# 0xPolygonZero/proof-protocol-decoder

Measured on NVIDIA B200. Metric: mpt_nodes_keccak_hashed_per_sec, higher is better.
Workload: dtype u64

## Files before the change

proof_protocol_decoder_b200/csrc/gpu_txn.cu:

```cuda
#include "host_pipeline.h"
#include "txn_tables.h"

namespace ppd {

bool gpu_txn_enabled() {
#ifdef PPD_HOSTPROF
  return false;
#else
  return gpu_parse_enabled() && gpu_dump_enabled() && getenv("PPD_HOST_TXN") == nullptr;
#endif
}

struct LoopBatcher {
  static const int MAX_STREAMS = 16, BMAX = (int)LOOP_BATCH_MAX;
  struct Req {
    txn::LoopTask task;
    uint32_t n_txns = 0;
    cudaEvent_t ready = nullptr, start = nullptr, done = nullptr, done_blocking = nullptr;
    bool launched = false;
    uint32_t launches = 0;
    cudaError_t err = cudaSuccess;
  };
  struct LoopStream {
    cudaStream_t st = nullptr;
    cudaEvent_t idle = nullptr;
    txn::LoopTask* tasks = nullptr;
  };
  int device = 0, n_streams = 0;
  LoopStream ls[MAX_STREAMS];
  std::mutex mu;
  std::condition_variable cv_work, cv_launched;
  std::deque<Req*> q;
  bool stop = false;
  std::thread th;

  void serve() {
#ifndef PPD_HOSTPROF
    cudaSetDevice(device);
    int next = 0;
    for (;;) {
      Req* batch[BMAX];
      int n = 0;
      {
        std::unique_lock<std::mutex> g(mu);
        cv_work.wait(g, [&] { return stop || !q.empty(); });
        if (stop && q.empty()) return;
      }
      int pick = -1;
      for (int k = 0; k < n_streams && pick < 0; k++) {
        const int s = (next + k) % n_streams;
        if (cudaEventQuery(ls[s].idle) == cudaSuccess) pick = s;
      }
      if (pick < 0) {
        pick = next;
        cudaEventSynchronize(ls[pick].idle);
      }
      next = (pick + 1) % n_streams;
      {
        std::lock_guard<std::mutex> g(mu);
        while (n < BMAX && !q.empty()) batch[n++] = q.front(), q.pop_front();
      }
      LoopStream& S = ls[pick];
      uint32_t max_txns = 0;
      bool any_shared = false;
      cudaError_t err = cudaSuccess;
      for (int k = 0; k < n; k++) {
        S.tasks[k] = batch[k]->task;
        max_txns = std::max(max_txns, batch[k]->n_txns);
        any_shared |= batch[k]->task.use_shared != 0;
        if (err == cudaSuccess) err = cudaStreamWaitEvent(S.st, batch[k]->ready, 0);
      }
      for (int k = 0; k < n && err == cudaSuccess; k++) err = cudaEventRecord(batch[k]->start, S.st);
      uint32_t launches = 0;
      if (err == cudaSuccess) {
        launches = launch_txn_loops(S.tasks, (uint32_t)n, max_txns, any_shared, S.st);
        err = cudaGetLastError();
      }
      for (int k = 0; k < n && err == cudaSuccess; k++) {
        err = cudaEventRecord(batch[k]->done, S.st);
        if (err == cudaSuccess) err = cudaEventRecord(batch[k]->done_blocking, S.st);
      }
      if (err == cudaSuccess) err = cudaEventRecord(S.idle, S.st);
      {
        std::lock_guard<std::mutex> g(mu);
        for (int k = 0; k < n; k++) batch[k]->launched = true, batch[k]->launches = launches, batch[k]->err = err;
      }
      cv_launched.notify_all();
    }
#endif
  }
};

LoopBatcher* loop_batcher_create(int device, int n_streams) {
#ifdef PPD_HOSTPROF
  return nullptr;
#else
  LoopBatcher* b = new LoopBatcher();
  b->device = device;
  b->n_streams = std::min(n_streams, (int)LoopBatcher::MAX_STREAMS);
  for (int k = 0; k < b->n_streams; k++) {
    LoopBatcher::LoopStream& S = b->ls[k];
    S.tasks = (txn::LoopTask*)pinned_alloc(sizeof(txn::LoopTask) * LoopBatcher::BMAX);
    if (!S.tasks || cudaStreamCreateWithFlags(&S.st, cudaStreamNonBlocking) != cudaSuccess ||
        cudaEventCreateWithFlags(&S.idle, cudaEventBlockingSync | cudaEventDisableTiming) != cudaSuccess || cudaEventRecord(S.idle, S.st) != cudaSuccess) {
      b->n_streams = k + 1;
      loop_batcher_destroy(b);
      return nullptr;
    }
  }
  b->th = std::thread([b] { b->serve(); });
  return b;
#endif
}
void loop_batcher_destroy(LoopBatcher* b) {
#ifndef PPD_HOSTPROF
  if (!b) return;
  if (b->th.joinable()) {
    {
      std::lock_guard<std::mutex> g(b->mu);
      b->stop = true;
    }
    b->cv_work.notify_all();
    b->th.join();
  }
  for (int k = 0; k < b->n_streams; k++) {
    if (b->ls[k].st) cudaStreamSynchronize(b->ls[k].st), cudaStreamDestroy(b->ls[k].st);
    if (b->ls[k].idle) cudaEventDestroy(b->ls[k].idle);
    if (b->ls[k].tasks) pinned_free(b->ls[k].tasks);
  }
  delete b;
#endif
}
uint32_t loop_batcher_run(LoopBatcher* b, const txn::View& v, uint32_t initial_state, uint32_t max_keys, cudaEvent_t ready, cudaEvent_t start,
                          cudaEvent_t done, cudaEvent_t done_blocking) {
#ifdef PPD_HOSTPROF
  return 0;
#else
  LoopBatcher::Req r;
  r.task.v = v, r.task.initial_state = initial_state, r.task.use_shared = txn_loop_uses_shared(max_keys);
  r.n_txns = v.n_txns, r.ready = ready, r.start = start, r.done = done, r.done_blocking = done_blocking;
  {
    std::lock_guard<std::mutex> g(b->mu);
    b->q.push_back(&r);
  }
  b->cv_work.notify_one();
  {
    std::unique_lock<std::mutex> g(b->mu);
    b->cv_launched.wait(g, [&] { return r.launched; });
  }
  CUDA_OK(r.err);
  return r.launches;
#endif
}

#ifndef PPD_HOSTPROF
namespace {

struct Carve2 {
  uint8_t* base;
  size_t off = 0;
  template <class T>
  T* take(size_t count) {
    off = (off + 255) & ~(size_t)255;
    T* r = reinterpret_cast<T*>(base + off);
    off += count * sizeof(T);
    return r;
  }
};

struct HookState {
  Lane* L;
  Job* J;
  TxnTables* T;
  const uint8_t* d_flat;
  size_t n_txns;
  TxnBases B{};
  txn::View v{};
  txn::JoinView j{};
  txn::AcctInit ai{};
  uint32_t table_slots = 0, n_pre_nodes = 0, cap_tail = 0;
  uint64_t* se = nullptr;
  uint32_t *bins_pre = nullptr, *bins_tail = nullptr;
  uint16_t* okeys = nullptr;
  txn::Withdrawal* d_withdrawals = nullptr;
  txn::AcctExport* d_export = nullptr;
  uint32_t* h_bins = nullptr;
  uint8_t* h_code_digests = nullptr;
};

void after_emit(void* arg, const ParseEmit& E) {
  HookState& H = *(HookState*)arg;
  Lane* L = H.L;
  Job& J = *H.J;
  TxnTables& T = *H.T;
  cudaStream_t st = L->st;
  const size_t n_nodes = J.dev.nodes, n_acct = J.dev.accounts, n_traces = T.traces.size();
  H.n_pre_nodes = (uint32_t)n_nodes;
  H.cap_tail = (uint32_t)T.est_nodes;
  TxnBases& B = H.B;
  B.dig_base = (uint32_t)((J.dev.keys + 31) & ~(size_t)31);
  B.txn_key_base = B.dig_base + 32u * T.n_msgs;
  B.key_cursor = B.txn_key_base + 12u * (uint32_t)H.n_txns;
  B.val_base = (uint32_t)((J.dev.vals + 3) & ~(size_t)3);
  B.rec_base = (uint32_t)n_acct;
  uint32_t table = 64;
  while (table < 2 * n_traces) table <<= 1;
  uint32_t jtable = 64;
  while (jtable < 2 * n_acct) jtable <<= 1;
  H.table_slots = table;
  txn::View& v = H.v;
  txn::JoinView& j = H.j;
  const size_t n_sorted = std::max<size_t>(n_nodes, T.est_nodes);
  const size_t pc_slow_n = (size_t)T.max_ops * txn::PATH_CAP;
  size_t pc_map_n = 64;
  while (pc_map_n < 2 * pc_slow_n) pc_map_n <<= 1;
  auto layout = [&](Carve2& c) {
    v.traces = c.take<txn::TxnTrace>(n_traces + 1);
    H.se = c.take<uint64_t>(2ull * T.n_msgs + 2);
    v.ops1 = c.take<txn::SOp>(T.n_ops1 + 1);
    v.ops2 = c.take<txn::SOp>(T.n_ops2 + 1);
    v.acct = c.take<txn::AcctState>(table);
    j.slot_owner = c.take<uint32_t>(jtable);
    j.slot_best = c.take<uint32_t>(jtable);
    j.join_storage = c.take<uint32_t>(n_acct + 1);
    j.join_root = c.take<uint32_t>(n_acct + 1);
    j.pre_flags = c.take<uint8_t>(n_acct + 1);
    v.pre_slot = c.take<uint32_t>(n_acct + 1);
    H.d_withdrawals = c.take<txn::Withdrawal>(T.withdrawals.size() + 1);
    H.d_export = c.take<txn::AcctExport>(T.needs_dummies() ? n_acct + 1 : 1);
    v.s.path_node = c.take<uint32_t>((size_t)T.max_ops * txn::PATH_CAP + 1);
    v.s.path_pc = c.take<uint32_t>((size_t)T.max_ops * txn::PATH_CAP + 1);
    v.s.path_depth = c.take<uint8_t>((size_t)T.max_ops * txn::PATH_CAP + 1);
    v.s.plen = c.take<uint8_t>(T.max_ops + 1);
    v.s.tnode = c.take<uint32_t>(T.max_ops + 1);
    v.s.tpc = c.take<uint32_t>(T.max_ops + 1);
    v.s.tdepth = c.take<uint8_t>(T.max_ops + 1);
    v.s.tkind = c.take<uint8_t>(T.max_ops + 1);
    v.s.key_hi = c.take<uint32_t>(T.max_ops + 1);
    v.s.pc_slow = c.take<txn::PathNode>(pc_slow_n + 1);
    v.s.pc_map = c.take<uint32_t>(pc_map_n);
    v.s.pc_map_key = c.take<uint32_t>(pc_map_n);
    v.cur = c.take<txn::Cursors>(1);
    H.bins_pre = c.take<uint32_t>(ORDER_MAX_BINS);
    H.bins_tail = c.take<uint32_t>(ORDER_MAX_BINS);
    H.okeys = c.take<uint16_t>(n_sorted + 16);
  };
  {
    Carve2 sz{nullptr};
    layout(sz);
    L->d_txn.reserve(sz.off + 256);
    Carve2 c{L->d_txn.as<uint8_t>()};
    layout(c);
  }
  v.nodes = E.nodes, v.level = E.level, v.key_pool = E.key_pool, v.val_pool = E.val_pool, v.hash_pool = E.hash_pool;
  v.child_pool = E.child_pool, v.accounts = E.accounts;
  v.cap_nodes = (uint32_t)(n_nodes + T.est_nodes), v.cap_children = (uint32_t)(J.dev.children + T.est_children);
  v.cap_keys = (uint32_t)std::min<size_t>(L->d_keys.cap, 0xfffffff0u);
  v.flat = H.d_flat, v.n_txns = (uint32_t)H.n_txns, v.n_traces = (uint32_t)n_traces, v.dig_base = B.dig_base;
  v.rec_base = B.rec_base, v.val_base = B.val_base;
  v.pre_flags = j.pre_flags;
  v.s.pc_fast = nullptr, v.s.pc_n_fast = 0, v.s.pc_n_slow = (uint32_t)pc_slow_n, v.s.pc_map_mask = (uint32_t)pc_map_n - 1, v.s.pc_count = &v.cur->pc_count;
  v.s.sh_ops = nullptr;
  v.s.a_nodes = &v.cur->n_nodes, v.s.a_children = &v.cur->n_children, v.s.a_keys = &v.cur->key_bytes, v.s.a_max_level = &v.cur->max_level;
  v.withdrawals = H.d_withdrawals, v.n_withdrawals = (uint32_t)T.withdrawals.size();
  lane_copy(L, H.d_withdrawals, T.withdrawals.data(), sizeof(txn::Withdrawal) * v.n_withdrawals);
  j.acct_list = E.acct_list, j.n_acct = (uint32_t)n_acct, j.table_mask = jtable - 1;
  lane_copy(L, v.traces, T.traces.data(), sizeof(txn::TxnTrace) * n_traces);
  lane_copy_flush(L);
  L->stats.h2d_bytes += (double)(sizeof(txn::TxnTrace) * n_traces);
  launch_txn_msgs(v, H.se, st);
  launch_keccak256_ranges(H.d_flat, H.se, T.n_msgs, E.key_pool + B.dig_base, st);
  L->stats.kernel_launches += 2, L->stats.key_hashes += T.n_msgs;
  for (size_t k = 0; k < T.code_write_traces.size(); k++) {
    const uint32_t m = T.traces[T.code_write_traces[k]].m_code;
    lane_copy(L, H.h_code_digests + 32 * k, E.key_pool + B.dig_base + 32ull * m, 32);
  }
  L->d_order.reserve(4ull * n_nodes + 16);
  CUDA_OK(cudaMemsetAsync(H.bins_pre, 0, 4ull * ORDER_MAX_BINS, st));
  launch_order_by_level_class(E.nodes, E.level, (uint32_t)n_nodes, ORDER_MAX_BINS, H.okeys, H.bins_pre, L->d_order.as<uint32_t>(), st);
  lane_copy(L, H.h_bins, H.bins_pre, 4ull * ORDER_MAX_BINS);
  L->stats.kernel_launches += 3, L->stats.d2h_bytes += 4.0 * ORDER_MAX_BINS;
}

void levels_from_bins(const uint32_t* bins, uint32_t n, std::vector<uint32_t>& level_start) {
  level_start.assign(1, 0);
  for (uint32_t l = 0; l < ORDER_MAX_BINS / 64; l++) {
    const uint32_t end = bins[64 * l + 63];
    level_start.push_back(end);
    if (end >= n) break;
  }
}

}
#endif

int gpu_block(ppd_ctx* c, Lane* L, Job& J, const uint8_t* flat, size_t len, uint8_t** out, size_t* out_len) {
#ifdef PPD_HOSTPROF
  return GPU_BLOCK_DECLINED;
#else
  BlockJob& b = J.blocks[0];
  if (!gpu_txn_enabled()) return GPU_BLOCK_DECLINED;
  {
    const char* e = getenv("PPD_GPU_PARSE_MIN_BYTES");
    const size_t min_bytes = e ? (size_t)atoll(e) : (size_t)512 << 10;
    if (b.compact.n < min_bytes || b.compact.n < 2) return GPU_BLOCK_DECLINED;
  }
  TxnTables& T = J.txn;
  PhaseTimer pt;
  if (!txn_tables_phase1(b, flat, len, T)) return GPU_BLOCK_DECLINED;
  pt.lap("t:tables1");
  cudaStream_t st = L->st;
  const ppd_stats stats0 = L->stats;
  const size_t wit_off = (size_t)(b.compact.p - flat);
  const size_t lead = (256 - (wit_off & 255)) & 255;
  L->d_flat.reserve(lead + len + 512);
  uint8_t* d_flat = L->d_flat.as<uint8_t>() + lead;
  L->tr_n = 0;
  trace_mark(L, "begin");
  upload_bytes(L, J, d_flat, flat, len);
  trace_mark(L, "uploaded");
  CUDA_OK(cudaMemsetAsync(d_flat + len, 0, 256, st));
  L->stats.h2d_bytes += (double)len;
  const size_t h_words = 2 * ORDER_MAX_BINS + sizeof(txn::Cursors) / 4 + 64;
  J.txn_host.resize(h_words + 8 * T.code_write_traces.size() + 8);
  HookState H;
  H.L = L, H.J = &J, H.T = &T, H.d_flat = d_flat, H.n_txns = b.txns.size();
  H.h_bins = J.txn_host.data();
  H.h_code_digests = reinterpret_cast<uint8_t*>(J.txn_host.data() + h_words);
  PreImageDeviceOnly X{};
  X.d_witness = d_flat + wit_off;
  X.extra_nodes = T.est_nodes, X.extra_children = T.est_children;
  X.extra_keys = 64 + 32ull * T.n_msgs + 12ull * b.txns.size() + 40ull * (T.n_ops1 + T.n_ops2) + 4096;
  X.extra_vals = 64 + T.val_writes + 8ull * b.txns.size();
  for (const TxnV& tx : b.txns) X.extra_vals += tx.byte_code.n + tx.new_receipt_node.n;
  X.extra_accounts = T.n_recs + 1;
  X.after_launch = after_emit, X.arg = &H;
  if (!gpu_pre_image(L, J, b, true, &c->parse_slots_sem, &X)) {
    L->stats = stats0;
    return GPU_BLOCK_DECLINED;
  }
  pt.lap("t:pre-image");
  trace_mark(L, "parsed");
  struct CD {
    HookState* H;
    TxnTables* T;
    std::vector<uint32_t> slot_of;
  } cd{&H, &T, {}};
  if (!T.code_write_traces.empty()) {
    cd.slot_of.assign(T.traces.size(), 0);
    for (size_t k = 0; k < T.code_write_traces.size(); k++) cd.slot_of[T.code_write_traces[k]] = (uint32_t)k;
  }
  auto code_digest = [](void* arg, uint32_t t) -> const uint8_t* {
    CD* x = (CD*)arg;
    return x->H->h_code_digests + 32ull * x->slot_of[t];
  };
  if (!txn_tables_phase2(b, flat, H.B, code_digest, &cd, T)) {
    L->stats = stats0;
    return GPU_BLOCK_DECLINED;
  }
  pt.lap("t:tables2");
  txn::View& v = H.v;
  const uint32_t n_ir = T.n_ir, n_seg = (uint32_t)T.seg_a.size(), n_touched = T.touched_begin[n_ir];
  const uint32_t n_pre = H.n_pre_nodes;
  const int n_dummies = (T.dummy_initial[0] >= 0) + (T.dummy_initial[1] >= 0) + (T.dummy_final >= 0);
  const size_t dummy_entries = J.dev.accounts + T.traces.size();
  const size_t seg_cap = n_seg + (size_t)n_dummies * (2 * dummy_entries + 32), lit_cap = T.lit.size() + (size_t)n_dummies * (36 * dummy_entries + 512);
  PVec<uint64_t>& big_off = J.big_off;
  PVec<uint32_t>& big_cap = J.big_cap;
  big_off.resize(n_ir + 1), big_cap.resize(n_ir + 1);
  size_t big_words = 0;
  for (uint32_t i = 0; i < n_ir; i++) {
    const uint32_t tn = T.touched_begin[i + 1] - T.touched_begin[i];
    big_off[i] = ~0ull, big_cap[i] = 0;
    if (tn <= 2 * IR_SET_MAX_UNIQ) continue;
    uint32_t cap = 1u << 14;
    while (cap < 2 * tn) cap <<= 1;
    big_off[i] = big_words, big_cap[i] = cap;
    big_words += 3ull * cap;
  }
  IrDumpPlanView P{};
  uint64_t* d_big_off;
  uint32_t* d_big_cap;
  uint32_t *d_seg_a, *d_seg_b, *d_seg_c, *d_seg_begin, *d_seg_end, *d_touched_begin, *d_touched, *d_ir_size;
  uint64_t* d_ir_base;
  uint8_t* d_lit;
  txn::TxnDesc* d_txns;
  auto plan_layout = [&](Carve2& cv) {
    d_txns = cv.take<txn::TxnDesc>(n_ir + 1);
    d_seg_a = cv.take<uint32_t>(seg_cap + 1), d_seg_b = cv.take<uint32_t>(seg_cap + 1), d_seg_c = cv.take<uint32_t>(seg_cap + 1);
    d_seg_begin = cv.take<uint32_t>(n_ir + 1), d_seg_end = cv.take<uint32_t>(n_ir + 1), d_touched_begin = cv.take<uint32_t>(n_ir + 1);
    d_lit = cv.take<uint8_t>(lit_cap + 16);
    d_ir_base = cv.take<uint64_t>(n_ir + 1);
    d_touched = cv.take<uint32_t>((size_t)n_touched + 16);
    P.seg_off = cv.take<uint32_t>(seg_cap + 1);
    d_ir_size = cv.take<uint32_t>(2ull * n_ir + 2);
    P.ir_nuniq = cv.take<uint32_t>(n_ir + 1);
    d_big_off = cv.take<uint64_t>(n_ir + 1), d_big_cap = cv.take<uint32_t>(n_ir + 1);
    P.big_scratch = cv.take<uint32_t>(big_words + 16);
    P.u_node = cv.take<uint32_t>((size_t)n_touched + 16), P.u_size = cv.take<uint32_t>((size_t)n_touched + 16), P.u_off = cv.take<uint32_t>((size_t)n_touched + 16);
  };
  {
    Carve2 sz{nullptr};
    plan_layout(sz);
    L->d_plan.reserve(sz.off + 256);
    Carve2 cv{L->d_plan.as<uint8_t>()};
    plan_layout(cv);
  }
  P.ir_size = d_ir_size, P.ir_flag = d_ir_size + n_ir;
  P.touched = d_touched, P.touched_begin = d_touched_begin, P.seg_a = d_seg_a, P.seg_b = d_seg_b, P.seg_c = d_seg_c, P.seg_begin = d_seg_begin;
  P.seg_end = d_seg_end;
  P.big_off = d_big_off, P.big_cap = d_big_cap;
  P.flat = d_flat, P.lit = d_lit, P.ir_base = d_ir_base;
  auto up = [&](void* dst, const void* src, size_t bytes) {
    if (!bytes) return;
    lane_copy(L, dst, src, bytes);
    L->stats.h2d_bytes += (double)bytes;
  };
  up(d_txns, T.txns.data(), sizeof(txn::TxnDesc) * T.txns.size());
  up(d_seg_a, T.seg_a.data(), 4ull * n_seg), up(d_seg_b, T.seg_b.data(), 4ull * n_seg), up(d_seg_c, T.seg_c.data(), 4ull * n_seg);
  up(d_touched_begin, T.touched_begin.data(), 4ull * (n_ir + 1));
  if (!n_dummies) up(d_seg_begin, T.seg_begin.data(), 4ull * (n_ir + 1)), up(d_seg_end, T.seg_end.data(), 4ull * (n_ir + 1));
  up(d_lit, T.lit.data(), T.lit.size());
  up(d_big_off, big_off.data(), 8ull * n_ir), up(d_big_cap, big_cap.data(), 4ull * n_ir);
  up(v.key_pool + H.B.txn_key_base, T.txn_keys.data(), T.txn_keys.size());
  lane_copy_flush(L);
  CUDA_OK(cudaMemsetAsync(d_touched, 0xff, 4ull * n_touched, st));
  v.txns = d_txns, v.touched = d_touched, v.seg_a = d_seg_a, v.seg_b = d_seg_b;
  std::vector<uint32_t> level_pre, level_tail;
  levels_from_bins(H.h_bins, n_pre, level_pre);
  L->d_ref.reserve(32ull * v.cap_nodes);
  L->d_ref_len.reserve(v.cap_nodes);
  L->d_counters.reserve(32);
  CUDA_OK(cudaMemsetAsync(L->d_counters.p, 0, 32, st));
  ArenaView V;
  V.nodes = v.nodes, V.key_pool = v.key_pool, V.val_pool = v.val_pool, V.hash_pool = v.hash_pool, V.child_pool = v.child_pool;
  V.accounts = v.accounts, V.ref = L->d_ref.as<uint8_t>(), V.ref_len = L->d_ref_len.as<uint8_t>();
  V.counters = L->d_counters.as<unsigned long long>();
  trace_mark(L, "plan_up");
  CUDA_OK(cudaEventRecord(L->ev0, st));
  for (size_t l = 0; l + 1 < level_pre.size(); l++) {
    launch_hash_level(V, L->d_order.as<uint32_t>(), level_pre[l], level_pre[l + 1], st);
    L->stats.kernel_launches++, L->stats.level_launches++;
  }
  CUDA_OK(cudaEventRecord(L->ev1, st));
  trace_mark(L, "pre_hashed");
  H.j.ref = V.ref;
  CUDA_OK(cudaMemsetAsync(H.j.slot_owner, 0xff, 4ull * (H.j.table_mask + 1), st));
  CUDA_OK(cudaMemsetAsync(H.j.slot_best, 0, 4ull * (H.j.table_mask + 1), st));
  CUDA_OK(cudaMemsetAsync(v.pre_slot, 0xff, 4ull * (H.j.n_acct + 1), st));
  txn::Cursors init;
  memset(&init, 0, sizeof init);
  init.n_nodes = n_pre, init.n_children = (uint32_t)J.dev.children, init.key_bytes = H.B.key_cursor;
  init.state_root = b.state_root, init.txn_root = NODE_EMPTY, init.receipt_root = NODE_EMPTY;
  launch_txn_init(v, init, H.table_slots, st);
  H.j.flag = &v.cur->flag;
  launch_join(H.j, st);
  H.ai = txn::AcctInit{H.table_slots - 1, b.state_root, H.j.join_storage, H.j.join_root};
  const uint32_t max_writes = T.max_trace_keys;
  L->stats.kernel_launches += 3 + launch_txn_prep(v, H.ai, T.n_ops1, T.n_ops2, max_writes, st);
#ifdef PPD_LOOP_PROF
  static unsigned long long* d_evlog = nullptr;
  static uint32_t* d_evcount = nullptr;
  const uint32_t ev_cap = 1u << 16;
  const char* ev_env = getenv("PPD_LOOP_EVLOG");
  if (ev_env) {
    if (!d_evlog) {
      CUDA_OK(cudaMalloc(&d_evlog, 16ull * ev_cap));
      CUDA_OK(cudaMalloc(&d_evcount, 4));
    }
    CUDA_OK(cudaMemsetAsync(d_evcount, 0, 4, st));
    v.evlog = d_evlog, v.evcount = d_evcount, v.ev_txn = (uint32_t)atoi(ev_env), v.ev_cap = ev_cap;
  }
#endif
  trace_mark(L, "prep");
  lane_copy_flush(L);
  CUDA_OK(cudaEventRecord(L->ev_ready, st));
  L->lease->release();
  L->stats.kernel_launches += loop_batcher_run(c->batcher, v, b.state_root, T.max_ops, L->ev_ready, L->ev_loop0, L->ev_loop1, L->ev_loop_done);
  {
    const auto tw = std::chrono::steady_clock::now();
    CUDA_OK(cudaEventSynchronize(L->ev_loop_done));
    L->stats.host_wait_ms += std::chrono::duration<double, std::milli>(std::chrono::steady_clock::now() - tw).count();
  }
  L->lease->acquire();
  st = L->st;
  trace_mark(L, "loop");
  L->d_order2.reserve(4ull * H.cap_tail + 16);
  CUDA_OK(cudaMemsetAsync(H.bins_tail, 0, 4ull * ORDER_MAX_BINS, st));
  launch_order_by_level_class(v.nodes, v.level, H.cap_tail, ORDER_MAX_BINS, H.okeys, H.bins_tail, L->d_order2.as<uint32_t>(), st, n_pre, &v.cur->n_nodes);
  CUDA_OK(cudaGetLastError());
  txn::Cursors* h_cur = reinterpret_cast<txn::Cursors*>(H.h_bins + 2 * ORDER_MAX_BINS);
  lane_copy(L, H.h_bins + ORDER_MAX_BINS, H.bins_tail, 4ull * ORDER_MAX_BINS);
  lane_copy(L, h_cur, v.cur, sizeof(txn::Cursors));
  L->stats.kernel_launches += 3, L->stats.d2h_bytes += 4.0 * ORDER_MAX_BINS + sizeof(txn::Cursors);
  trace_mark(L, "tail_order");
  lane_sync(L);
  pt.lap("t:loop");
#ifdef PPD_LOOP_PROF
  if (ev_env && strchr(ev_env, ':')) {
    uint32_t n_ev = 0;
    CUDA_OK(cudaMemcpy(&n_ev, d_evcount, 4, cudaMemcpyDeviceToHost));
    n_ev = std::min(n_ev, ev_cap);
    std::vector<unsigned long long> ev(2ull * n_ev);
    if (n_ev) CUDA_OK(cudaMemcpy(ev.data(), d_evlog, 16ull * n_ev, cudaMemcpyDeviceToHost));
    if (FILE* f = fopen(strchr(ev_env, ':') + 1, "w")) {
      fprintf(f, "clock,thread,event\n");
      for (uint32_t k = 0; k < n_ev; k++) fprintf(f, "%llu,%llu,%llu\n", ev[2 * k], ev[2 * k + 1] >> 16, ev[2 * k + 1] & 0xffff);
      fclose(f);
    }
  }
#endif
  {
    float ms = 0;
    CUDA_OK(cudaEventElapsedTime(&ms, L->ev0, L->ev1));
    L->stats.gpu_ms += ms;
    CUDA_OK(cudaEventElapsedTime(&ms, L->ev_loop0, L->ev_loop1));
    L->stats.txn_gpu_ms += ms;
  }
  if (getenv("PPD_TIMING")) {
    const unsigned long long* pc = h_cur->phase_clocks;
    fprintf(stderr, "[ppd]   loop phases (Mclk): setup %.2f | walks %.2f | announce %.2f | storage tries up %.2f | records %.2f | state trie up %.2f | root nodes %.2f\n",
            pc[0] / 1e6, pc[1] / 1e6, pc[2] / 1e6, pc[3] / 1e6, pc[4] / 1e6, pc[5] / 1e6, pc[6] / 1e6);
  }
  if (h_cur->flag || h_cur->max_level >= ORDER_MAX_BINS / 64) {
    if (getenv("PPD_TIMING")) fprintf(stderr, "[ppd] device txn loop flag %u at txn %u (max level %u): host path\n", h_cur->flag, h_cur->flag_txn, h_cur->max_level);
    L->stats = stats0;
    L->has_last_parse = false;
    return GPU_BLOCK_DECLINED;
  }
  if (n_dummies) {
    const size_t n_acct = J.dev.accounts, n_tr = T.traces.size();
    const size_t w_export = (sizeof(txn::AcctExport) * (n_acct + 1) + 3) / 4, w_table = (sizeof(txn::AcctState) * H.table_slots + 3) / 4, w_dig = 8 * (n_tr + 1);
    J.txn_export.resize(w_export + w_table + w_dig + 16);
    txn::AcctExport* h_export = reinterpret_cast<txn::AcctExport*>(J.txn_export.data());
    txn::AcctState* h_table = reinterpret_cast<txn::AcctState*>(J.txn_export.data() + w_export);
    uint8_t* h_dig = reinterpret_cast<uint8_t*>(J.txn_export.data() + w_export + w_table);
    launch_acct_export(v, H.j, H.d_export, st);
    CUDA_OK(cudaGetLastError());
    lane_copy(L, h_export, H.d_export, sizeof(txn::AcctExport) * n_acct);
    lane_copy(L, h_table, v.acct, sizeof(txn::AcctState) * H.table_slots);
    lane_copy(L, h_dig, v.key_pool + H.B.dig_base, 32ull * n_tr);
    L->stats.kernel_launches += 1, L->stats.d2h_bytes += (double)(sizeof(txn::AcctExport) * n_acct + sizeof(txn::AcctState) * H.table_slots + 32ull * n_tr);
    lane_sync(L);
    const size_t seg0 = T.seg_a.size(), lit0 = T.lit.size();
    txn_tables_dummies(b, flat, *h_cur, h_export, (uint32_t)n_acct, h_table, H.table_slots, h_dig, T);
    if (T.seg_a.size() > seg_cap || T.lit.size() > lit_cap) fail(PPD_ERR_BAD_ARGUMENT, "dummy entries exceed their plan space");
    up(d_seg_a + seg0, T.seg_a.data() + seg0, 4ull * (T.seg_a.size() - seg0)), up(d_seg_b + seg0, T.seg_b.data() + seg0, 4ull * (T.seg_b.size() - seg0));
    up(d_seg_c + seg0, T.seg_c.data() + seg0, 4ull * (T.seg_c.size() - seg0));
    up(d_lit + lit0, T.lit.data() + lit0, T.lit.size() - lit0);
    up(d_seg_begin, T.seg_begin.data(), 4ull * (n_ir + 1)), up(d_seg_end, T.seg_end.data(), 4ull * (n_ir + 1));
    lane_copy_flush(L);
    pt.lap("t:dummies");
  }
  const uint32_t n_total = h_cur->n_nodes, n_tail = n_total - n_pre;
  levels_from_bins(H.h_bins + ORDER_MAX_BINS, n_tail, level_tail);
  trace_mark(L, "host_resumed");
  CUDA_OK(cudaEventRecord(L->ev0, st));
  for (size_t l = 0; l + 1 < level_tail.size(); l++) {
    launch_hash_level(V, L->d_order2.as<uint32_t>(), level_tail[l], level_tail[l + 1], st);
    L->stats.kernel_launches++, L->stats.level_launches++;
  }
  CUDA_OK(cudaEventRecord(L->ev1, st));
  trace_mark(L, "tail_hashed");
  CUDA_OK(cudaEventRecord(L->ev_loop0, st));
  launch_ir_size(V, P, n_ir, st);
  CUDA_OK(cudaEventRecord(L->ev_loop1, st));
  CUDA_OK(cudaGetLastError());
  J.plan.resize(2ull * n_ir + 8);
  uint32_t* h_sizes = J.plan.data();
  unsigned long long* h_counters = reinterpret_cast<unsigned long long*>(H.h_bins);
  lane_copy(L, h_sizes, d_ir_size, 8ull * n_ir);
  lane_copy(L, h_counters, L->d_counters.p, 24);
  L->stats.kernel_launches += 1, L->stats.d2h_bytes += 8.0 * n_ir + 24;
  trace_mark(L, "ir_sized");
  lane_sync(L);
  pt.lap("t:sweep+size");
  {
    float ms = 0;
    CUDA_OK(cudaEventElapsedTime(&ms, L->ev0, L->ev1));
    L->stats.gpu_ms += ms;
    CUDA_OK(cudaEventElapsedTime(&ms, L->ev_loop0, L->ev_loop1));
    L->stats.dump_gpu_ms += ms;
  }
  L->stats.nodes_hashed += h_counters[0], L->stats.node_permutations += h_counters[1], L->stats.node_bytes += h_counters[2];
  L->stats.arena_nodes += n_total;
  L->stats.levels += level_pre.size() + level_tail.size() - 2;
  for (size_t m = 0; m < T.traces.size(); m++) {
    const txn::TxnTrace& tr = T.traces[m];
    L->stats.key_permutations += 1 + tr.n_reads + tr.n_writes + ((tr.flags & txn::TRF_MIN_KEYS) ? tr.n_writes : 0);
    if ((tr.flags & PPD_TR_CODE_WRITE) && !(tr.flags & PPD_TR_CODE_READ)) L->stats.key_permutations += tr.code_len / 136 + 1;
  }
  L->stats.marks_on_gpu += T.n_items;
  L->stats.txn_loops_on_gpu += 1;
  L->has_last = true, L->last_view = V;
  L->last_level_start = level_pre, L->last_level_start2 = level_tail, L->last_n_msgs = T.n_msgs;
  L->last_msg_data = d_flat, L->last_msg_se = H.se, L->last_digest_out = v.key_pool + H.B.dig_base;
  L->last_txn = H.v, L->last_join = H.j, L->last_ai = H.ai, L->last_init = init, L->last_table_slots = H.table_slots;
  L->last_n_ops1 = T.n_ops1, L->last_n_ops2 = T.n_ops2, L->last_max_writes = max_writes, L->last_n_touched = n_touched, L->last_max_keys = T.max_ops;
  L->last_plan = P, L->last_n_ir = n_ir, L->has_last_txn = true;
  L->last_cap_tail = H.cap_tail, L->last_bins_tail = H.bins_tail, L->last_okeys = H.okeys;
  uint64_t total = 8;
  PVec<uint64_t>& ir_base = J.ir_base;
  ir_base.resize(n_ir);
  for (uint32_t i = 0; i < n_ir; i++) {
    if (h_sizes[n_ir + i]) {
      if (getenv("PPD_TIMING")) fprintf(stderr, "[ppd] IR %u cannot be laid out on the device: host path\n", i);
      L->stats = stats0;
      L->has_last = L->has_last_parse = L->has_last_txn = false;
      return GPU_BLOCK_DECLINED;
    }
    ir_base[i] = total;
    total += h_sizes[i];
  }
  Out o;
  uint8_t* pinned = total >= ((size_t)1 << 20) ? out_pool().take(total) : nullptr;
  if (!pinned) o.need(total);
  uint8_t* dst = pinned ? pinned : o.p;
  L->d_out.reserve(total + 64);
  L->last_out_bytes = total;
  up(d_ir_base, ir_base.data(), 8ull * n_ir);
  launch_store_u32x2(L->d_out.as<uint32_t>(), PPD_IR_DUMP_MAGIC, n_ir, st);
  L->stats.h2d_bytes += 8;
  lane_copy_flush(L);
  trace_mark(L, "host_resumed2");
  CUDA_OK(cudaEventRecord(L->ev0, st));
  launch_ir_emit(V, P, n_ir, L->d_out.as<uint8_t>(), st);
  CUDA_OK(cudaEventRecord(L->ev1, st));
  trace_mark(L, "ir_emitted");
  CUDA_OK(cudaGetLastError());
  L->stats.kernel_launches += 1;
  if (pinned) {
    const auto tw = std::chrono::steady_clock::now();
    cudaError_t e = cudaMemcpyAsync(dst, L->d_out.p, total, cudaMemcpyDeviceToHost, st);
    trace_mark(L, "downloaded");
    if (e == cudaSuccess) e = cudaEventRecord(L->ev_sync, st);
    if (e == cudaSuccess) e = cudaEventSynchronize(L->ev_sync);
    L->stats.host_wait_ms += std::chrono::duration<double, std::milli>(std::chrono::steady_clock::now() - tw).count();
    if (e != cudaSuccess) {
      out_pool().give_back(pinned);
      throw Fail{PPD_ERR_CUDA, std::string("IR dump copy: ") + cudaGetErrorString(e)};
    }
  } else {
    J.out_stage.resize(total);
    CUDA_OK(cudaMemcpyAsync(J.out_stage.data(), L->d_out.p, total, cudaMemcpyDeviceToHost, st));
    lane_sync(L);
    memcpy(o.p, J.out_stage.data(), total);
    o.n = total;
  }
  L->stats.d2h_bytes += (double)total;
  {
    float ms = 0;
    CUDA_OK(cudaEventElapsedTime(&ms, L->ev0, L->ev1));
    L->stats.dump_gpu_ms += ms;
  }
  pt.lap("t:emit+copy");
  trace_mark(L, "end");
  trace_flush(L);
  if (pinned) {
    *out = pinned, *out_len = total;
  } else {
    *out = o.give(out_len);
  }
  return GPU_BLOCK_DONE;
#endif
}

}
```

proof_protocol_decoder_b200/csrc/host_pipeline.h:

```cpp
#pragma once
#include <cuda_runtime.h>
#include <sys/mman.h>

#include <algorithm>
#include <atomic>
#include <chrono>
#include <condition_variable>
#include <cstdio>
#include <cstdlib>
#include <cstring>
#include <deque>
#include <map>
#include <memory>
#include <mutex>
#include <string>
#include <thread>
#include <unordered_set>
#include <unordered_map>
#include <vector>

#include "../../include/ppd_b200.h"
#include "arena.h"
#include "devbuf.h"
#include "flat_maps.h"
#include "host_arena.h"
#include "ppd_kernels.h"
#include "txn_tables.h"

namespace ppd {

static const uint8_t EMPTY_CODE_HASH[32] = {0xc5, 0xd2, 0x46, 0x01, 0x86, 0xf7, 0x23, 0x3c, 0x92, 0x7e, 0x7d, 0xb2, 0xdc, 0xc7, 0x03, 0xc0,
                                            0xe5, 0x00, 0xb6, 0x53, 0xca, 0x82, 0x27, 0x3b, 0x7b, 0xfa, 0xd8, 0x04, 0x5d, 0x85, 0xa4, 0x70};
static const uint8_t EMPTY_TRIE_HASH[32] = {0x56, 0xe8, 0x1f, 0x17, 0x1b, 0xcc, 0x55, 0xa6, 0xff, 0x83, 0x45, 0xe6, 0x92, 0xc0, 0xf8, 0x6e,
                                            0x5b, 0x48, 0xe0, 0x1b, 0x99, 0x6c, 0xad, 0xc0, 0x01, 0x62, 0x2f, 0xb5, 0xe3, 0x63, 0xb4, 0x21};

struct Job;
void job_delete(Job*);
void* pinned_alloc(size_t n);
void pinned_free(void* p);

struct Lane {
  cudaStream_t st = nullptr;
  cudaEvent_t ev0 = nullptr, ev1 = nullptr;
  cudaEvent_t ev_sync = nullptr;
  ppd_stats stats{};
  DevBuf d_nodes, d_order, d_keys, d_vals, d_hashes, d_children, d_accounts, d_ref, d_ref_len, d_counters;
  DevBuf d_msg, d_msg_off, d_digest;
  DevBuf d_plan, d_out;
  DevBuf d_wit, d_pa, d_pb, d_pc;
  DevBuf d_level, d_okeys, d_obins;
  DevBuf d_flat, d_txn, d_order2;
  cudaEvent_t ev_loop0 = nullptr, ev_loop1 = nullptr;
  uint32_t* h_parse = nullptr;
  bool has_last_parse = false;
  ParseBounds last_bounds{};
  ParseEmit last_emit{};
  uint32_t* last_ins_pos = nullptr;
  uint32_t last_n_code = 0;
  size_t last_val_bytes = 0;
  Job* job = nullptr;
  bool has_last = false;
  ArenaView last_view{};
  std::vector<uint32_t> last_level_start, last_level_start2;
  uint32_t last_n_msgs = 0;
  const uint8_t* last_msg_data = nullptr;
  const uint64_t* last_msg_se = nullptr;
  uint8_t* last_digest_out = nullptr;
  bool has_last_txn = false;
  txn::View last_txn{};
  txn::JoinView last_join{};
  txn::AcctInit last_ai{};
  txn::Cursors last_init{};
  uint32_t last_table_slots = 0, last_n_ops1 = 0, last_n_ops2 = 0, last_max_writes = 0, last_n_touched = 0, last_n_ir = 0, last_cap_tail = 0, last_max_keys = 0;
  uint32_t* last_bins_tail = nullptr;
  uint16_t* last_okeys = nullptr;
  IrDumpPlanView last_plan{};
  size_t last_out_bytes = 0;
  std::vector<cudaEvent_t> tr_ev;
  std::vector<const char*> tr_label;
  std::vector<double> tr_host_ms;
  size_t tr_n = 0;
  int id = 0;
  CopyBatch copies;
  cudaStream_t own_st = nullptr;
  struct StreamLease* lease = nullptr;
  txn::LoopTask* h_task = nullptr;
  cudaEvent_t ev_ready = nullptr, ev_loop_done = nullptr;
};

struct Slots {
  std::mutex mu;
  std::condition_variable cv;
  int free_slots;
  explicit Slots(int n) : free_slots(n) {}
  void acquire() {
    std::unique_lock<std::mutex> g(mu);
    cv.wait(g, [&] { return free_slots > 0; });
    free_slots--;
  }
  void release() {
    {
      std::lock_guard<std::mutex> g(mu);
      free_slots++;
    }
    cv.notify_one();
  }
};
struct SlotGuard {
  Slots* s;
  explicit SlotGuard(Slots* s_, double* wait_ms = nullptr) : s(s_) {
    if (!s) return;
    const auto t0 = std::chrono::steady_clock::now();
    s->acquire();
    if (wait_ms) *wait_ms += std::chrono::duration<double, std::milli>(std::chrono::steady_clock::now() - t0).count();
  }
  void done() {
    if (s) s->release();
    s = nullptr;
  }
  ~SlotGuard() { done(); }
};
constexpr int PARSE_SLOTS = 8;

}

namespace ppd {
struct StreamPool {
  std::mutex mu;
  std::condition_variable cv;
  std::vector<cudaStream_t> all, free_;
  cudaStream_t acquire(double* wait_ms) {
    const auto t0 = std::chrono::steady_clock::now();
    std::unique_lock<std::mutex> g(mu);
    cv.wait(g, [&] { return !free_.empty(); });
    cudaStream_t s = free_.back();
    free_.pop_back();
    if (wait_ms) *wait_ms += std::chrono::duration<double, std::milli>(std::chrono::steady_clock::now() - t0).count();
    return s;
  }
  void release(cudaStream_t s) {
    {
      std::lock_guard<std::mutex> g(mu);
      free_.push_back(s);
    }
    cv.notify_one();
  }
};
struct StreamLease {
  StreamPool* pool;
  Lane* L;
  bool held = false;
  StreamLease(StreamPool* p, Lane* l) : pool(p), L(l) {
    L->lease = this;
    acquire();
  }
  void acquire() {
    if (!pool || held) return;
    L->st = pool->acquire(&L->stats.host_wait_ms);
    held = true;
  }
  void release() {
    if (!pool || !held) return;
    lane_copy_flush_fwd(L);
    pool->release(L->st);
    L->st = L->own_st;
    held = false;
  }
  ~StreamLease() {
    release();
    L->lease = nullptr;
  }
  static void lane_copy_flush_fwd(Lane* l);
};
struct LoopBatcher;
LoopBatcher* loop_batcher_create(int device, int n_streams);
void loop_batcher_destroy(LoopBatcher* b);
uint32_t loop_batcher_run(LoopBatcher* b, const txn::View& v, uint32_t initial_state, uint32_t max_keys, cudaEvent_t ready, cudaEvent_t start,
                          cudaEvent_t done, cudaEvent_t done_blocking);
}

struct ppd_ctx {
  int device = 0;
  ppd::StreamPool* pool = nullptr;
  ppd::LoopBatcher* batcher = nullptr;
  ppd::Slots parse_slots_sem{ppd::PARSE_SLOTS};
  cudaStream_t st = nullptr;
  cudaEvent_t ev0 = nullptr, ev1 = nullptr;
  std::string err;
  std::mutex err_mu;
  ppd_stats stats{};
  std::vector<ppd::Lane*> lanes;
  size_t last_lanes_used = 0;
  ppd::DevBuf d_keys, d_vals, d_ref, d_ref_len, d_counters;
  ppd::DevBuf d_msg, d_msg_off, d_digest;
  ppd::DevBuf d_build[12];
};

namespace ppd {

void stats_reset(ppd_ctx* c);
void lane_sync(Lane* l);
void lane_copy(Lane* l, void* dst, const void* src, size_t bytes);
void lane_copy_flush(Lane* l);
bool trace_on();
void trace_mark(Lane* l, const char* label);
void trace_flush(Lane* l);

struct KeyHasher {
  PVec<uint8_t> data;
  std::vector<uint64_t> off{0};
  PVec<H256> digest;
  std::vector<uint64_t> lens;
  PVec<uint64_t> se;
  KeyHasher() {
    data.alloc_fn = pinned_alloc, data.free_fn = pinned_free;
    digest.alloc_fn = pinned_alloc, digest.free_fn = pinned_free;
    se.alloc_fn = pinned_alloc, se.free_fn = pinned_free;
  }
  void reset() {
    data.clear(), digest.clear(), lens.clear(), se.clear();
    off.assign(1, 0);
  }
  uint32_t add(const uint8_t* p, size_t n) {
    size_t at = data.size(), padded = (n + 3) & ~(size_t)3;
    data.resize(at + padded);
    memcpy(data.data() + at, p, n);
    memset(data.data() + at + n, 0, padded - n);
    uint32_t idx = (uint32_t)lens.size();
    lens.push_back(n);
    off.push_back(data.size());
    return idx;
  }
  void run(Lane* c);
};

struct Span {
  const uint8_t* p = nullptr;
  uint32_t n = 0;
};
struct WNode {
  uint32_t pos;
  uint8_t op, flags;
  uint16_t unused = 0;
  int32_t first_child;
  int32_t next_sibling;
  uint32_t aux;
};

struct WCursor {
  const uint8_t* p;
  size_t n, pos = 0;
  uint8_t read_byte() {
    if (pos >= n) fail(PPD_ERR_UNEXPECTED_END_OF_STREAM, "read_byte at end of stream");
    return p[pos++];
  }
  bool cbor_head(uint8_t& major, uint64_t& arg) {
    if (pos >= n) return false;
    uint8_t b = p[pos++];
    major = b >> 5;
    uint8_t ai = b & 31;
    if (ai < 24) {
      arg = ai;
      return true;
    }
    if (ai > 27) return false;
    size_t w = (size_t)1 << (ai - 24);
    if (n - pos < w) return false;
    arg = 0;
    for (size_t i = 0; i < w; i++) arg = (arg << 8) | p[pos++];
    return true;
  }
  Span cbor_bytes(int err) {
    uint8_t major;
    uint64_t len;
    if (!cbor_head(major, len) || major != 2 || len > n - pos) fail(err, "bad CBOR byte string");
    Span s{p + pos, (uint32_t)len};
    pos += len;
    return s;
  }
  uint64_t cbor_uint(uint64_t max) {
    uint8_t major;
    uint64_t v;
    if (!cbor_head(major, v) || major != 0 || v > max) fail(PPD_ERR_INVALID_BYTES_FOR_TYPE, "bad CBOR unsigned integer");
    return v;
  }
};

inline uint32_t compact_key_nibbles(Span k, uint8_t* out) {
  if (k.n == 0) return 0;
  uint32_t c = 0;
  if (k.n == 1) {
    out[c++] = k.p[0] & 15;
    return c;
  }
  bool odd = k.p[0] & 1;
  uint32_t m = k.n - 1;
  if (2 * m > 64 + 1) fail(PPD_ERR_KEY_ERROR, "compact key longer than 64 nibbles");
  for (uint32_t i = 0; i + 1 < m; i++) {
    out[c++] = k.p[1 + i] >> 4;
    out[c++] = k.p[1 + i] & 15;
  }
  out[c++] = k.p[m] >> 4;
  if (!odd) out[c++] = k.p[m] & 15;
  return c;
}

inline void check_key_length(Span k) {
  if (k.n >= 2 && 2 * (k.n - 1) > 64 + 1) fail(PPD_ERR_KEY_ERROR, "compact key longer than 64 nibbles");
}

struct Witness {
  const uint8_t* bytes = nullptr;
  size_t len = 0;
  uint8_t version = 0;
  std::vector<WNode> ins;
  int32_t root = -1;

  Span key(const WNode& x) const {
    WCursor c{bytes, len, x.pos};
    return c.cbor_bytes(PPD_ERR_INVALID_BYTE_VECTOR);
  }
  Span leaf_value(const WNode& x) const {
    WCursor c{bytes, len, x.pos};
    c.cbor_bytes(PPD_ERR_INVALID_BYTE_VECTOR);
    return c.cbor_bytes(PPD_ERR_INVALID_BYTE_VECTOR);
  }
  Span code(const WNode& x) const { return key(x); }
  const uint8_t* hash(const WNode& x) const { return bytes + x.pos; }
  void account(const WNode& x, Span& key_out, uint64_t& nonce, Span& balance) const {
    WCursor c{bytes, len, x.pos};
    key_out = c.cbor_bytes(PPD_ERR_INVALID_BYTE_VECTOR);
    c.pos++;
    nonce = (x.flags & 4) ? c.cbor_uint(~0ull) : 0;
    balance = (x.flags & 8) ? c.cbor_bytes(PPD_ERR_INVALID_BYTE_VECTOR) : Span{};
  }
};
void parse_witness(const uint8_t* w, size_t n, Witness& out);

struct TrieItem {
  uint32_t koff, klen;
  uint8_t kind;
  uint32_t a1, a2;
};

struct TraceV {
  const uint8_t* addr;
  uint8_t flags;
  const uint8_t *balance = nullptr, *nonce = nullptr;
  uint32_t n_reads = 0, n_writes = 0;
  const uint8_t *reads = nullptr, *writes = nullptr;
  const uint8_t* code_read = nullptr;
  Span code_write;
  uint32_t m_addr = 0, m_reads = 0, m_writes_full = 0, m_writes_min = 0, m_code = 0;
};
struct TxnV {
  std::vector<TraceV> traces;
  Span byte_code, new_txn_node, new_receipt_node;
  uint64_t gas_used = 0;
};
struct FlatReader {
  const uint8_t* p;
  size_t n, pos = 0;
  void need(size_t k) {
    if (n - pos < k) fail(PPD_ERR_BAD_FLAT_INPUT, "flat block truncated");
  }
  uint8_t u8() {
    need(1);
    return p[pos++];
  }
  uint32_t u32() {
    need(4);
    uint32_t v;
    memcpy(&v, p + pos, 4);
    pos += 4;
    return v;
  }
  uint64_t u64() {
    need(8);
    uint64_t v;
    memcpy(&v, p + pos, 8);
    pos += 8;
    return v;
  }
  const uint8_t* raw(size_t k) {
    need(k);
    const uint8_t* r = p + pos;
    pos += k;
    return r;
  }
  Span bytes() {
    uint32_t k = u32();
    return Span{raw(k), k};
  }
};

struct IrPlan {
  uint64_t txn_before = 0, gas_before = 0, gas_after = 0;
  bool has_signed_txn = false;
  Span signed_txn;
  bool has_withdrawals = false;
  uint32_t state_sub = NODE_EMPTY, txn_sub = NODE_EMPTY, receipt_sub = NODE_EMPTY;
  std::vector<std::pair<H256, uint32_t>> storage_subs;
  std::vector<uint32_t> touched;
  uint32_t root_state = 0, root_txn = 0, root_receipt = 0;
  std::map<H256, Span> code;
};

struct BlockJob {
  Span compact;
  uint32_t pre_image_kind = 0;
  Span direct;
  std::vector<uint8_t> compact_owned;
  std::vector<H256> direct_keep;
  std::vector<TxnV> txns;
  std::unordered_map<H256, Span, H256Hasher> resolved_code;
  std::vector<std::pair<const uint8_t*, const uint8_t*>> withdrawals;
  std::vector<uint32_t> m_withdrawal_addr;
  const uint8_t* checkpoint = nullptr;
  Span b_meta, b_hashes;
  Witness wit;
  std::vector<uint32_t> m_inline_code;
  std::map<H256, Span> pre_code;
  uint32_t state_root = NODE_EMPTY;
  H256Map storage;
  struct PreAccount {
    H256 haddr;
    uint32_t rec;
    bool storage_nonempty;
    bool witnesses_storage = false;
    uint32_t own_root = NODE_EMPTY;
  };
  bool storage_partial = false;
  bool pre_image_built = false;
  std::vector<PreAccount> pre_accounts;
  H256Map pre_with_storage;
  FlatMapU32 root_of;
  std::unordered_map<int32_t, uint32_t> storage_root_of_instr;
  bool have_empty_form = false;
  bool pre_image_on_gpu = false;
  uint32_t empty_form = NODE_EMPTY;
  std::vector<IrPlan> irs;
  int status = PPD_OK;
  std::string err;
};

void read_flat_block(const uint8_t* p, size_t n, BlockJob& b);
void direct_to_compact(BlockJob& b);
void direct_filter_storage(BlockJob& b);
uint32_t u256_sig(const uint8_t* be);
void rlp_str(std::vector<uint8_t>& out, const uint8_t* p, size_t n);
void rlp_u256(std::vector<uint8_t>& out, const uint8_t* be);
struct RlpItem {
  bool is_list;
  const uint8_t* payload;
  size_t payload_len, total_len;
};
bool rlp_item(const uint8_t* p, size_t n, RlpItem& it);
bool is_legacy_receipt(const uint8_t* p, size_t n);

struct Job {
  HostArena A;
  KeyHasher kh;
  std::vector<BlockJob> blocks;
  PVec<uint8_t> ref, ref_len;
  PVec<uint32_t> order;
  PVec<uint32_t> plan;
  PVec<uint8_t> out_stage;
  bool refs_on_host = false;
  struct Resident {
    size_t nodes = 0, keys = 0, vals = 0, hashes = 0, children = 0, accounts = 0;
  } dev;
  bool pools_on_host = true;
  PVec<uint32_t> acct_list, code_list;
  PVec<uint8_t> wit_stage;
  std::vector<HostArena::MarkItem> mark_items;
  std::vector<HostArena::BatchItem> batch_items;
  std::vector<uint32_t> haddr_keys, haddr_leaves;
  PVec<H256> code_digest;
  TxnTables txn;
  PVec<uint32_t> txn_host;
  PVec<uint32_t> txn_export;
  PVec<uint64_t> ir_base, big_off;
  PVec<uint32_t> big_cap;
  std::vector<uint32_t> stamp;
  uint32_t serial = 0;
  Job() {
    plan.alloc_fn = pinned_alloc, plan.free_fn = pinned_free;
    out_stage.alloc_fn = pinned_alloc, out_stage.free_fn = pinned_free;
    A.set_allocator(pinned_alloc, pinned_free);
    ref.alloc_fn = ref_len.alloc_fn = pinned_alloc, ref.free_fn = ref_len.free_fn = pinned_free;
    order.alloc_fn = pinned_alloc, order.free_fn = pinned_free;
    A.level.alloc_fn = pinned_alloc, A.level.free_fn = pinned_free;
    acct_list.alloc_fn = code_list.alloc_fn = pinned_alloc, acct_list.free_fn = code_list.free_fn = pinned_free;
    code_digest.alloc_fn = pinned_alloc, code_digest.free_fn = pinned_free;
    wit_stage.alloc_fn = pinned_alloc, wit_stage.free_fn = pinned_free;
    txn.set_allocator(pinned_alloc, pinned_free);
    txn_host.alloc_fn = pinned_alloc, txn_host.free_fn = pinned_free;
    txn_export.alloc_fn = pinned_alloc, txn_export.free_fn = pinned_free;
    ir_base.alloc_fn = pinned_alloc, ir_base.free_fn = pinned_free;
    big_off.alloc_fn = pinned_alloc, big_off.free_fn = pinned_free, big_cap.alloc_fn = pinned_alloc, big_cap.free_fn = pinned_free;
  }
  void reset(size_t n_blocks) {
    dev = Resident{};
    pools_on_host = true;
    A.clear();
    kh.reset();
    blocks.clear();
    blocks.resize(n_blocks);
    ref.clear(), ref_len.clear(), order.clear();
    serial = 0;
  }
};

Job& job_of(Lane* l, size_t n_blocks);
Lane* lane_of(ppd_ctx* c, size_t w);
void lane_delete(Lane* l);
void collect_witness_messages(Job& J, BlockJob& b);
void collect_messages(Job& J, BlockJob& b);
uint32_t root_node_for(Job& J, BlockJob& b, uint32_t trie_root);
void build_pre_image(Job& J, BlockJob& b);
void join_storage_by_root(Lane* L, Job& J, BlockJob& b);
bool gpu_parse_enabled();
struct PreImageDeviceOnly {
  const uint8_t* d_witness;
  size_t extra_nodes, extra_children, extra_keys, extra_vals, extra_accounts;
  void (*after_launch)(void* arg, const ParseEmit& E);
  void* arg;
};
bool gpu_pre_image(Lane* L, Job& J, BlockJob& b, bool check_version = true, Slots* slots = nullptr, const PreImageDeviceOnly* dev_only = nullptr);
void upload_bytes(Lane* L, Job& J, uint8_t* dst, const uint8_t* src, size_t n);
void verify_gpu_pre_image(Lane* L, Job& J, BlockJob& b);
void shape_block(Job& J, BlockJob& b);
void sweep(Lane* c, Job& J, bool refs_to_host = true);
void fetch_refs(Lane* c, Job& J);
void fetch_pools(Lane* c, Job& J);

struct PhaseTimer {
  bool on = getenv("PPD_TIMING") != nullptr;
  std::chrono::steady_clock::time_point t = std::chrono::steady_clock::now();
  void lap(const char* what) {
    if (!on) return;
    auto now = std::chrono::steady_clock::now();
    fprintf(stderr, "[ppd] %-10s %8.3f ms\n", what, std::chrono::duration<double, std::milli>(now - t).count());
    t = now;
  }
};
struct SectionTimer {
  bool on = getenv("PPD_TIMING") != nullptr;
  double acc[8] = {0, 0, 0, 0, 0, 0, 0, 0};
  std::chrono::steady_clock::time_point t;
  void start() {
    if (on) t = std::chrono::steady_clock::now();
  }
  void stop(int k) {
    if (!on) return;
    auto now = std::chrono::steady_clock::now();
    acc[k] += std::chrono::duration<double, std::milli>(now - t).count();
    t = now;
  }
  void report(const char* const* names, int n) {
    if (!on) return;
    for (int k = 0; k < n; k++) fprintf(stderr, "[ppd]   %-12s %8.3f ms\n", names[k], acc[k]);
  }
};

struct Out {
  uint8_t* p = nullptr;
  size_t n = 0, cap = 0;
  Out() {}
  Out(const Out&) = delete;
  Out& operator=(const Out&) = delete;
  Out(Out&& o) noexcept : p(o.p), n(o.n), cap(o.cap) { o.p = nullptr, o.n = o.cap = 0; }
  ~Out() { free(p); }
  void need(size_t k) {
    if (n + k <= cap) return;
    size_t nc = cap ? cap * 2 : 4096;
    while (nc < n + k) nc *= 2;
    uint8_t* q;
    if (nc >= (8u << 20)) {
      nc = (nc + (2u << 20) - 1) & ~(size_t)((2u << 20) - 1);
      q = (uint8_t*)aligned_alloc(2u << 20, nc);
      if (q) {
        madvise(q, nc, MADV_HUGEPAGE);
        if (n) memcpy(q, p, n);
        free(p);
      }
    } else {
      q = (uint8_t*)realloc(p, nc);
    }
    if (!q) fail(PPD_ERR_BAD_ARGUMENT, "out of host memory");
    p = q, cap = nc;
  }
  void u8(uint8_t v) {
    need(1);
    p[n++] = v;
  }
  void u32(uint32_t v) {
    need(4);
    memcpy(p + n, &v, 4);
    n += 4;
  }
  void u64(uint64_t v) {
    need(8);
    memcpy(p + n, &v, 8);
    n += 8;
  }
  void raw(const uint8_t* q, size_t k) {
    need(k);
    if (k) memcpy(p + n, q, k);
    n += k;
  }
  void span(Span s) {
    u32(s.n);
    raw(s.p, s.n);
  }
  void u256(uint64_t v) {
    need(32);
    memset(p + n, 0, 24);
    for (int i = 0; i < 8; i++) p[n + 31 - i] = (uint8_t)(v >> (8 * i));
    n += 32;
  }
  uint8_t* give(size_t* len) {
    uint8_t* r = p ? p : (uint8_t*)malloc(1);
    *len = n;
    p = nullptr, n = cap = 0;
    return r;
  }
};

struct Stamp {
  std::vector<uint32_t> v;
  uint32_t serial = 0;
};

void dump_ir(const Job& J, const BlockJob& b, IrPlan& p, Stamp& st, Out& o);
void dump_blocks(Job& J, uint8_t** outs, size_t* out_lens, unsigned max_workers);
unsigned host_threads();

template <class F>
void parallel_for(size_t n, unsigned workers, F f) {
  if (workers > n) workers = (unsigned)n;
  if (workers <= 1) {
    for (size_t i = 0; i < n; i++) f(i, 0u);
    return;
  }
  std::atomic<size_t> next{0};
  std::atomic<bool> failed{false};
  Fail first{PPD_OK, ""};
  std::mutex mu;
  auto body = [&](unsigned w) {
    for (;;) {
      size_t i = next.fetch_add(1);
      if (i >= n || failed.load()) return;
      try {
        f(i, w);
      } catch (const Fail& e) {
        std::lock_guard<std::mutex> g(mu);
        if (!failed.exchange(true)) first = e;
      } catch (const std::exception& e) {
        std::lock_guard<std::mutex> g(mu);
        if (!failed.exchange(true)) first = Fail{PPD_ERR_BAD_ARGUMENT, e.what()};
      }
    }
  };
  std::vector<std::thread> th;
  for (unsigned w = 1; w < workers; w++) th.emplace_back(body, w);
  body(0);
  for (auto& t : th) t.join();
  if (failed.load()) throw first;
}

struct OutPool {
  struct Entry {
    uint8_t* p;
    size_t cap;
    bool in_use;
  };
  std::mutex mu;
  std::vector<Entry> entries;
  size_t total = 0;
  size_t limit() {
    static size_t v = [] {
      const char* e = getenv("PPD_PINNED_OUT_MB");
      return (size_t)(e ? atoll(e) : 12288) << 20;
    }();
    return v;
  }
  uint8_t* take(size_t n) {
#ifdef PPD_HOSTPROF
    return nullptr;
#else
    std::lock_guard<std::mutex> g(mu);
    Entry* best = nullptr;
    for (Entry& e : entries)
      if (!e.in_use && e.cap >= n && (!best || e.cap < best->cap)) best = &e;
    if (best) {
      best->in_use = true;
      return best->p;
    }
    size_t cap = (n + (n >> 3) + (8u << 20) - 1) & ~(size_t)((8u << 20) - 1);
    if (total + cap > limit()) {
      for (size_t i = 0; i < entries.size() && total + cap > limit();)
        if (!entries[i].in_use) {
          cudaFreeHost(entries[i].p);
          total -= entries[i].cap;
          entries.erase(entries.begin() + i);
        } else {
          i++;
        }
      if (total + cap > limit()) return nullptr;
    }
    void* p = nullptr;
    if (cudaHostAlloc(&p, cap, cudaHostAllocPortable) != cudaSuccess) return nullptr;
    entries.push_back({(uint8_t*)p, cap, true});
    total += cap;
    return (uint8_t*)p;
#endif
  }
  bool give_back(void* p) {
    std::lock_guard<std::mutex> g(mu);
    for (Entry& e : entries)
      if (e.p == p) {
        e.in_use = false;
        return true;
      }
    return false;
  }
};
OutPool& out_pool();

bool gpu_txn_enabled();
enum { GPU_BLOCK_DECLINED = 0, GPU_BLOCK_DONE = 1 };
int gpu_block(ppd_ctx* c, Lane* L, Job& J, const uint8_t* flat, size_t len, uint8_t** out, size_t* out_len);
bool gpu_dump_enabled();
enum { DUMP_ON_HOST = 0, DUMP_DONE = 1 };
int gpu_dump_block(ppd_ctx* c, Lane* L, Job& J, uint8_t** out, size_t* out_len);

}
```

proof_protocol_decoder_b200/csrc/ppd_host.cu:

```cuda
#include <time.h>

#include "host_pipeline.h"
#ifdef PPD_HOSTPROF
#include "../../tools/hostprof_stub.h"
#endif

using namespace ppd;

namespace ppd {

#ifdef PPD_HOSTPROF
void* pinned_alloc(size_t n) { return malloc(n); }
void pinned_free(void* p) { free(p); }
#else
void* pinned_alloc(size_t n) {
  void* p = nullptr;
  return cudaHostAlloc(&p, n, cudaHostAllocDefault) == cudaSuccess ? p : nullptr;
}
void pinned_free(void* p) { cudaFreeHost(p); }
#endif

void stats_reset(ppd_ctx* c) { c->stats = ppd_stats{}; }

void StreamLease::lane_copy_flush_fwd(Lane* l) { lane_copy_flush(l); }
void lane_copy_flush(Lane* l) {
#ifndef PPD_HOSTPROF
  if (!l->copies.n) return;
  launch_copy_segments(l->copies, l->st);
  CUDA_OK(cudaGetLastError());
  l->stats.kernel_launches += 1;
  l->copies.n = 0;
#endif
}
void lane_copy(Lane* l, void* dst, const void* src, size_t bytes) {
  if (!bytes) return;
  if (l->copies.n == CopyBatch::MAX) lane_copy_flush(l);
  CopyBatch& b = l->copies;
  b.dst[b.n] = dst, b.src[b.n] = src, b.bytes[b.n] = bytes, b.n++;
}

void lane_sync(Lane* l) {
  lane_copy_flush(l);
  const auto t0 = std::chrono::steady_clock::now();
  CUDA_OK(cudaEventRecord(l->ev_sync, l->st));
  CUDA_OK(cudaEventSynchronize(l->ev_sync));
  l->stats.host_wait_ms += std::chrono::duration<double, std::milli>(std::chrono::steady_clock::now() - t0).count();
}

namespace {
struct TraceState {
  FILE* f = nullptr;
  cudaEvent_t base = nullptr;
  std::chrono::steady_clock::time_point host0;
  std::mutex mu;
  unsigned seq = 0;
};
TraceState& trace_state() {
  static TraceState* t = [] {
    TraceState* s = new TraceState;
#ifndef PPD_HOSTPROF
    const char* path = getenv("PPD_TRACE");
    if (path && *path && (s->f = fopen(path, "w")) != nullptr) {
      if (cudaEventCreate(&s->base) != cudaSuccess || cudaEventRecord(s->base, 0) != cudaSuccess || cudaEventSynchronize(s->base) != cudaSuccess) {
        fclose(s->f);
        s->f = nullptr;
      }
      s->host0 = std::chrono::steady_clock::now();
      if (s->f) fprintf(s->f, "lane,block,label,device_ms,host_ms\n");
    }
#endif
    return s;
  }();
  return *t;
}
}
bool trace_on() { return trace_state().f != nullptr; }
void trace_mark(Lane* l, const char* label) {
#ifndef PPD_HOSTPROF
  TraceState& t = trace_state();
  if (!t.f) return;
  if (l->tr_n == l->tr_ev.size()) {
    cudaEvent_t e;
    CUDA_OK(cudaEventCreate(&e));
    l->tr_ev.push_back(e), l->tr_label.push_back(label), l->tr_host_ms.push_back(0);
  }
  CUDA_OK(cudaEventRecord(l->tr_ev[l->tr_n], l->st));
  l->tr_label[l->tr_n] = label;
  l->tr_host_ms[l->tr_n] = std::chrono::duration<double, std::milli>(std::chrono::steady_clock::now() - t.host0).count();
  l->tr_n++;
#endif
}
void trace_flush(Lane* l) {
#ifndef PPD_HOSTPROF
  TraceState& t = trace_state();
  if (!t.f || !l->tr_n) return;
  std::lock_guard<std::mutex> g(t.mu);
  const unsigned seq = t.seq++;
  for (size_t k = 0; k < l->tr_n; k++) {
    float ms = 0;
    if (cudaEventSynchronize(l->tr_ev[k]) != cudaSuccess || cudaEventElapsedTime(&ms, t.base, l->tr_ev[k]) != cudaSuccess) ms = -1;
    fprintf(t.f, "%d,%u,%s,%.4f,%.4f\n", l->id, seq, l->tr_label[k], ms, l->tr_host_ms[k]);
  }
  fflush(t.f);
  l->tr_n = 0;
#endif
}

void KeyHasher::run(Lane* c) {
  size_t n = lens.size();
  digest.resize(n);
  if (!n) return;
#ifdef PPD_HOSTPROF
  for (size_t i = 0; i < n; i++) hostprof::keccak256(data.data() + off[i], lens[i], digest[i].b);
  return;
#endif
  se.resize(2 * n);
  for (size_t i = 0; i < n; i++) se[2 * i] = off[i], se[2 * i + 1] = off[i] + lens[i];
  c->d_msg.reserve(data.size() + 16);
  c->d_msg_off.reserve(se.size() * 8);
  c->d_digest.reserve(n * 32);
  CUDA_OK(cudaMemcpyAsync(c->d_msg.p, data.data(), data.size(), cudaMemcpyHostToDevice, c->st));
  CUDA_OK(cudaMemcpyAsync(c->d_msg_off.p, se.data(), se.size() * 8, cudaMemcpyHostToDevice, c->st));
  launch_keccak256_ranges(c->d_msg.as<uint8_t>(), c->d_msg_off.as<uint64_t>(), (uint32_t)n, c->d_digest.as<uint8_t>(), c->st);
  CUDA_OK(cudaGetLastError());
  CUDA_OK(cudaMemcpyAsync(digest.data(), c->d_digest.p, n * 32, cudaMemcpyDeviceToHost, c->st));
  lane_sync(c);
  c->stats.key_hashes += n;
  for (size_t i = 0; i < n; i++) c->stats.key_permutations += lens[i] / 136 + 1;
  c->stats.h2d_bytes += (double)(data.size() + se.size() * 8);
  c->stats.d2h_bytes += (double)(n * 32);
  c->stats.kernel_launches += 1;
}

void job_delete(Job* j) { delete j; }
Job& job_of(Lane* l, size_t n_blocks) {
  if (!l->job) l->job = new Job();
  l->job->reset(n_blocks);
  return *l->job;
}

Lane* lane_of(ppd_ctx* c, size_t w) {
  while (c->lanes.size() <= w) {
    std::unique_ptr<Lane> l(new Lane());
    l->id = (int)c->lanes.size();
#ifndef PPD_HOSTPROF
    CUDA_OK(cudaStreamCreateWithFlags(&l->st, cudaStreamNonBlocking));
    l->own_st = l->st;
    l->h_task = (txn::LoopTask*)pinned_alloc(sizeof(txn::LoopTask));
    if (!l->h_task) fail(PPD_ERR_BAD_ARGUMENT, "out of page-locked memory");
    CUDA_OK(cudaEventCreateWithFlags(&l->ev_ready, cudaEventDisableTiming));
    CUDA_OK(cudaEventCreateWithFlags(&l->ev_loop_done, cudaEventBlockingSync | cudaEventDisableTiming));
    CUDA_OK(cudaEventCreate(&l->ev0));
    CUDA_OK(cudaEventCreate(&l->ev1));
    CUDA_OK(cudaEventCreateWithFlags(&l->ev_sync, cudaEventBlockingSync | cudaEventDisableTiming));
    CUDA_OK(cudaEventCreate(&l->ev_loop0));
    CUDA_OK(cudaEventCreate(&l->ev_loop1));
#endif
    c->lanes.push_back(l.release());
  }
  return c->lanes[w];
}
void lane_delete(Lane* l) {
#ifndef PPD_HOSTPROF
  DevBuf* bufs[] = {&l->d_nodes, &l->d_order,  &l->d_keys,     &l->d_vals, &l->d_hashes,  &l->d_children, &l->d_accounts,
                    &l->d_ref,   &l->d_ref_len, &l->d_counters, &l->d_msg,  &l->d_msg_off, &l->d_digest,
                    &l->d_plan,  &l->d_out,     &l->d_wit,      &l->d_pa,   &l->d_pb,      &l->d_pc,
                    &l->d_level, &l->d_okeys,   &l->d_obins,    &l->d_flat, &l->d_txn,     &l->d_order2};
  for (DevBuf* b : bufs) b->release();
  if (l->h_parse) pinned_free(l->h_parse);
  for (cudaEvent_t e : l->tr_ev) cudaEventDestroy(e);
  if (l->h_task) pinned_free(l->h_task);
  if (l->ev_ready) cudaEventDestroy(l->ev_ready);
  if (l->ev_loop_done) cudaEventDestroy(l->ev_loop_done);
  if (l->ev0) cudaEventDestroy(l->ev0);
  if (l->ev1) cudaEventDestroy(l->ev1);
  if (l->ev_sync) cudaEventDestroy(l->ev_sync);
  if (l->ev_loop0) cudaEventDestroy(l->ev_loop0);
  if (l->ev_loop1) cudaEventDestroy(l->ev_loop1);
  if (l->st) cudaStreamDestroy(l->st);
#endif
  if (l->job) job_delete(l->job);
  delete l;
}

void sweep(Lane* c, Job& J, bool refs_to_host) {
  HostArena& A = J.A;
  uint32_t n = (uint32_t)A.nodes.size();
  J.ref.resize(32ull * n);
  J.ref_len.resize(n);
  J.refs_on_host = true;
  if (!n) return;
#ifdef PPD_HOSTPROF
  memset(J.ref.data(), 0, 32ull * n);
  memset(J.ref_len.data(), 32, n);
  return;
#endif
  uint32_t n_levels = 0;
  for (uint32_t i = 0; i < n; i++) n_levels = std::max<uint32_t>(n_levels, A.level[i] + 1u);
  std::vector<uint32_t> level_start(n_levels + 1, 0);
  for (uint32_t i = 0; i < n; i++) level_start[A.level[i] + 1u]++;
  for (uint32_t l = 0; l < n_levels; l++) level_start[l + 1] += level_start[l];
  const bool device_order = 64u * n_levels <= ORDER_MAX_BINS;
  PVec<uint32_t>& order = J.order;
  if (!device_order) {
    auto node_class = [&](uint32_t i) -> uint32_t {
      const NodeRec& r = A.nodes[i];
      uint32_t kind = r.w0 & 0xff;
      if (kind == NK_BRANCH) return 40 + ((uint32_t)__builtin_popcount(r.a1 & 0xffff) - 1 & 15);
      if (kind == NK_ROOT) return 56;
      uint32_t perms = 1;
      if (kind == NK_LEAF) {
        uint32_t nl = (r.w0 >> 16) & 0xff;
        perms = ((nl < 2 ? 1 : 2 + (nl >> 1)) + r.a2 + 6) / 136 + 1;
      }
      return kind * 8 + (perms > 8 ? 7 : perms - 1);
    };
    order.resize(n);
    std::vector<uint8_t> cls(n);
    std::vector<uint32_t> bucket((size_t)n_levels * 64 + 1, 0);
    for (uint32_t i = 0; i < n; i++) {
      cls[i] = (uint8_t)node_class(i);
      bucket[(size_t)A.level[i] * 64 + cls[i] + 1]++;
    }
    for (size_t k = 0; k + 1 < bucket.size(); k++) bucket[k + 1] += bucket[k];
    for (uint32_t i = 0; i < n; i++) order[bucket[(size_t)A.level[i] * 64 + cls[i]]++] = i;
  }
  const Job::Resident& R = J.dev;
  c->d_nodes.reserve_keep(16ull * n, 16ull * R.nodes, c->st);
  c->d_order.reserve(4ull * n);
  c->d_keys.reserve_keep(A.key_pool.size() + 16, R.keys, c->st);
  c->d_vals.reserve_keep(A.val_pool.size() + 16, R.vals, c->st);
  c->d_hashes.reserve_keep(A.hash_pool.size() + 32, R.hashes, c->st);
  c->d_children.reserve_keep(4ull * A.child_pool.size() + 16, 4ull * R.children, c->st);
  c->d_accounts.reserve_keep(sizeof(AccountRec) * A.accounts.size() + 16, sizeof(AccountRec) * R.accounts, c->st);
  c->d_ref.reserve(32ull * n);
  c->d_ref_len.reserve(n);
  c->d_counters.reserve(32);
  auto up = [&](DevBuf& d, const void* src, size_t bytes, size_t resident = 0) {
    if (bytes <= resident) return;
    CUDA_OK(cudaMemcpyAsync(d.as<uint8_t>() + resident, (const uint8_t*)src + resident, bytes - resident, cudaMemcpyHostToDevice, c->st));
    c->stats.h2d_bytes += (double)(bytes - resident);
  };
  up(c->d_nodes, A.nodes.data(), 16ull * n, 16ull * R.nodes);
  if (device_order) {
    c->d_level.reserve_keep(2ull * n + 16, 2ull * R.nodes, c->st);
    c->d_okeys.reserve(2ull * n + 16);
    c->d_obins.reserve(4ull * ORDER_MAX_BINS);
    up(c->d_level, A.level.data(), 2ull * n, 2ull * R.nodes);
    CUDA_OK(cudaMemsetAsync(c->d_obins.p, 0, 4ull * 64 * n_levels, c->st));
    launch_order_by_level_class(c->d_nodes.as<NodeRec>(), c->d_level.as<uint16_t>(), n, 64 * n_levels, c->d_okeys.as<uint16_t>(),
                                c->d_obins.as<uint32_t>(), c->d_order.as<uint32_t>(), c->st);
    c->stats.kernel_launches += 3;
  } else {
    up(c->d_order, order.data(), 4ull * n);
  }
  up(c->d_keys, A.key_pool.data(), A.key_pool.size(), R.keys);
  up(c->d_vals, A.val_pool.data(), A.val_pool.size(), R.vals);
  up(c->d_hashes, A.hash_pool.data(), A.hash_pool.size(), R.hashes);
  up(c->d_children, A.child_pool.data(), 4ull * A.child_pool.size(), 4ull * R.children);
  up(c->d_accounts, A.accounts.data(), sizeof(AccountRec) * A.accounts.size(), sizeof(AccountRec) * R.accounts);
  CUDA_OK(cudaMemsetAsync(c->d_counters.p, 0, 32, c->st));
  ArenaView V;
  V.nodes = c->d_nodes.as<NodeRec>();
  V.key_pool = c->d_keys.as<uint8_t>();
  V.val_pool = c->d_vals.as<uint8_t>();
  V.hash_pool = c->d_hashes.as<uint8_t>();
  V.child_pool = c->d_children.as<uint32_t>();
  V.accounts = c->d_accounts.as<AccountRec>();
  V.ref = c->d_ref.as<uint8_t>();
  V.ref_len = c->d_ref_len.as<uint8_t>();
  V.counters = c->d_counters.as<unsigned long long>();
  CUDA_OK(cudaEventRecord(c->ev0, c->st));
  for (uint32_t l = 0; l < n_levels; l++) {
    launch_hash_level(V, c->d_order.as<uint32_t>(), level_start[l], level_start[l + 1], c->st);
    c->stats.kernel_launches++;
    c->stats.level_launches++;
  }
  CUDA_OK(cudaGetLastError());
  CUDA_OK(cudaEventRecord(c->ev1, c->st));
  unsigned long long counters[3] = {0, 0, 0};
  c->has_last = true;
  c->last_view = V;
  c->last_level_start = level_start;
  c->last_level_start2.clear();
  c->last_msg_data = nullptr;
  c->has_last_txn = false;
  c->last_n_msgs = (uint32_t)J.kh.lens.size();
  J.refs_on_host = refs_to_host;
  if (refs_to_host) {
    CUDA_OK(cudaMemcpyAsync(J.ref.data(), c->d_ref.p, 32ull * n, cudaMemcpyDeviceToHost, c->st));
    CUDA_OK(cudaMemcpyAsync(J.ref_len.data(), c->d_ref_len.p, n, cudaMemcpyDeviceToHost, c->st));
  }
  CUDA_OK(cudaMemcpyAsync(counters, c->d_counters.p, 24, cudaMemcpyDeviceToHost, c->st));
  lane_sync(c);
  float ms = 0;
  CUDA_OK(cudaEventElapsedTime(&ms, c->ev0, c->ev1));
  c->stats.gpu_ms += ms;
  c->stats.nodes_hashed += counters[0];
  c->stats.node_permutations += counters[1];
  c->stats.node_bytes += counters[2];
  c->stats.arena_nodes += n;
  c->stats.levels += n_levels;
  if (refs_to_host) c->stats.d2h_bytes += 33.0 * n;
}

void fetch_refs(Lane* c, Job& J) {
  if (J.refs_on_host) return;
  size_t n = J.A.nodes.size();
  CUDA_OK(cudaMemcpyAsync(J.ref.data(), c->d_ref.p, 32ull * n, cudaMemcpyDeviceToHost, c->st));
  CUDA_OK(cudaMemcpyAsync(J.ref_len.data(), c->d_ref_len.p, n, cudaMemcpyDeviceToHost, c->st));
  lane_sync(c);
  c->stats.d2h_bytes += 33.0 * n;
  J.refs_on_host = true;
}

void fetch_pools(Lane* c, Job& J) {
  if (J.pools_on_host) return;
  if (J.dev.vals) CUDA_OK(cudaMemcpyAsync(J.A.val_pool.data(), c->d_vals.p, J.dev.vals, cudaMemcpyDeviceToHost, c->st));
  if (J.dev.hashes) CUDA_OK(cudaMemcpyAsync(J.A.hash_pool.data(), c->d_hashes.p, J.dev.hashes, cudaMemcpyDeviceToHost, c->st));
  lane_sync(c);
  c->stats.d2h_bytes += (double)(J.dev.vals + J.dev.hashes);
  J.pools_on_host = true;
}

}

namespace {

template <class F>
int guarded(ppd_ctx* c, F f) {
  if (!c) return PPD_ERR_BAD_ARGUMENT;
  try {
#ifndef PPD_HOSTPROF
    CUDA_OK(cudaSetDevice(c->device));
#endif
    f();
    return PPD_OK;
  } catch (const Fail& e) {
    c->err = e.msg;
    return e.code;
  } catch (const std::exception& e) {
    c->err = e.what();
    return PPD_ERR_BAD_ARGUMENT;
  }
}

}

namespace ppd {
OutPool& out_pool() {
  static OutPool* p = new OutPool();
  return *p;
}
}

namespace {

void decode_one_inner(ppd_ctx* c, Lane* L, const uint8_t* flat, size_t len, uint8_t** out, size_t* out_len, int* status, unsigned dump_workers);
static double thread_cpu_ms() {
  timespec ts;
  clock_gettime(CLOCK_THREAD_CPUTIME_ID, &ts);
  return 1e3 * (double)ts.tv_sec + 1e-6 * (double)ts.tv_nsec;
}
void decode_one(ppd_ctx* c, Lane* L, const uint8_t* flat, size_t len, uint8_t** out, size_t* out_len, int* status, unsigned dump_workers) {
  const double t0 = thread_cpu_ms();
  decode_one_inner(c, L, flat, len, out, out_len, status, dump_workers);
  L->stats.host_busy_ms += thread_cpu_ms() - t0;
}
void decode_one_inner(ppd_ctx* c, Lane* L, const uint8_t* flat, size_t len, uint8_t** out, size_t* out_len, int* status, unsigned dump_workers) {
  *out = nullptr, *out_len = 0;
  StreamLease lease(c->pool, L);
  for (int on_device = gpu_txn_enabled() ? 1 : 0; on_device >= 0; on_device--) {
    PhaseTimer pt;
    Job& J = job_of(L, 1);
    BlockJob& b = J.blocks[0];
    try {
      read_flat_block(flat, len, b);
      pt.lap("read-flat");
      if (b.pre_image_kind == 2) {
        if (on_device) continue;
        direct_to_compact(b);
        pt.lap("direct");
      }
      if (on_device) {
        if (gpu_block(c, L, J, flat, len, out, out_len) == GPU_BLOCK_DONE) {
          *status = PPD_OK;
          return;
        }
        continue;
      }
      if (gpu_parse_enabled()) gpu_pre_image(L, J, b, true, &c->parse_slots_sem);
      collect_messages(J, b);
      pt.lap("parse");
      J.kh.run(L);
      pt.lap("keyhash");
      if (!b.pre_image_built) build_pre_image(J, b);
      if (b.pre_image_kind == 2)
        direct_filter_storage(b);
      else if (b.storage_partial)
        join_storage_by_root(L, J, b);
      shape_block(J, b);
      pt.lap("shape");
      sweep(L, J, !gpu_dump_enabled());
      pt.lap("sweep");
      if (gpu_dump_block(c, L, J, out, out_len) == DUMP_ON_HOST) {
        fetch_refs(L, J);
        fetch_pools(L, J);
        dump_blocks(J, out, out_len, dump_workers);
      }
      pt.lap("dump");
      *status = PPD_OK;
      return;
    } catch (const std::bad_alloc&) {
      *status = PPD_ERR_BAD_FLAT_INPUT;
      std::lock_guard<std::mutex> g(c->err_mu);
      c->err = "out of memory while reading the block";
      return;
    } catch (const Fail& e) {
      if (e.code == PPD_ERR_CUDA) throw;
      *status = e.code;
      std::lock_guard<std::mutex> g(c->err_mu);
      c->err = e.msg;
      return;
    }
  }
}

void add_stats(ppd_stats& a, const ppd_stats& b) {
  a.nodes_hashed += b.nodes_hashed, a.node_permutations += b.node_permutations, a.key_hashes += b.key_hashes;
  a.key_permutations += b.key_permutations, a.node_bytes += b.node_bytes, a.arena_nodes += b.arena_nodes;
  a.levels = std::max(a.levels, b.levels);
  a.gpu_ms += b.gpu_ms, a.h2d_bytes += b.h2d_bytes, a.d2h_bytes += b.d2h_bytes, a.kernel_launches += b.kernel_launches;
  a.witnesses_on_gpu += b.witnesses_on_gpu, a.witness_instructions += b.witness_instructions, a.witness_bytes += b.witness_bytes;
  a.parse_gpu_ms += b.parse_gpu_ms, a.level_launches += b.level_launches, a.marks_on_gpu += b.marks_on_gpu;
  a.txn_loops_on_gpu += b.txn_loops_on_gpu, a.txn_gpu_ms += b.txn_gpu_ms, a.dump_gpu_ms += b.dump_gpu_ms;
  a.host_busy_ms += b.host_busy_ms, a.host_wait_ms += b.host_wait_ms;
}

static const size_t MAX_LANES = 64, LANES_CAP = 128;
static size_t max_lanes() {
  static const size_t n = [] {
    const char* e = getenv("PPD_MAX_LANES");
    const long v = e ? atol(e) : (long)MAX_LANES;
    return (size_t)(v < 1 ? 1 : v > (long)LANES_CAP ? (long)LANES_CAP : v);
  }();
  return n;
}

void decode_blocks(ppd_ctx* c, const uint8_t* const* flats, const size_t* lens, size_t n, uint8_t** outs, size_t* out_lens, int* statuses,
                   ppd_block_done_fn done = nullptr, void* user = nullptr) {
  stats_reset(c);
  if (!n) return;
  const size_t n_lanes = std::min(n, max_lanes());
  const unsigned workers = (unsigned)std::min<size_t>(host_threads(), n_lanes);
  for (size_t w = 0; w < n_lanes; w++) {
    Lane* L = lane_of(c, w);
    L->stats = ppd_stats{};
    L->has_last = false;
    L->has_last_parse = false;
    L->has_last_txn = false;
  }
  const unsigned dump_workers = std::max(1u, host_threads() / workers);
  for (size_t i = 0; i < n; i++) outs[i] = nullptr, out_lens[i] = 0, statuses[i] = PPD_OK;
  parallel_for(n_lanes, workers, [&](size_t lane, unsigned) {
#ifndef PPD_HOSTPROF
    CUDA_OK(cudaSetDevice(c->device));
#endif
    for (size_t i = lane; i < n; i += n_lanes) {
      decode_one(c, c->lanes[lane], flats[i], lens[i], &outs[i], &out_lens[i], &statuses[i], dump_workers);
      if (done) {
        uint8_t* o = outs[i];
        outs[i] = nullptr;
        done(user, i, statuses[i], o, out_lens[i]);
      }
    }
  });
  c->last_lanes_used = n_lanes;
  for (size_t w = 0; w < n_lanes; w++) add_stats(c->stats, c->lanes[w]->stats);
}

}

extern "C" {

int ppd_ctx_create(int device, ppd_ctx** out) {
  if (!out) return PPD_ERR_BAD_ARGUMENT;
  *out = nullptr;
#ifdef PPD_HOSTPROF
  *out = new ppd_ctx();
  return PPD_OK;
#endif
  setenv("CUDA_DEVICE_MAX_CONNECTIONS", "32", 0);
  int count = 0;
  if (cudaGetDeviceCount(&count) != cudaSuccess || device < 0 || device >= count) return PPD_ERR_CUDA;
  ppd_ctx* c = new ppd_ctx();
  c->device = device;
  if (cudaSetDevice(device) != cudaSuccess || cudaStreamCreateWithFlags(&c->st, cudaStreamNonBlocking) != cudaSuccess ||
      cudaEventCreate(&c->ev0) != cudaSuccess || cudaEventCreate(&c->ev1) != cudaSuccess) {
    delete c;
    return PPD_ERR_CUDA;
  }
  constexpr int MAIN_STREAMS = 22, LOOP_STREAMS = 8;
  c->pool = new StreamPool();
  for (int k = 0; k < MAIN_STREAMS; k++) {
    cudaStream_t s = nullptr;
    if (cudaStreamCreateWithFlags(&s, cudaStreamNonBlocking) != cudaSuccess) {
      ppd_ctx_destroy(c);
      return PPD_ERR_CUDA;
    }
    c->pool->all.push_back(s), c->pool->free_.push_back(s);
  }
  c->batcher = loop_batcher_create(device, LOOP_STREAMS);
  if (!c->batcher) {
    ppd_ctx_destroy(c);
    return PPD_ERR_CUDA;
  }
  *out = c;
  return PPD_OK;
}

void ppd_ctx_destroy(ppd_ctx* c) {
  if (!c) return;
#ifdef PPD_HOSTPROF
  for (Lane* l : c->lanes) lane_delete(l);
  delete c;
  return;
#endif
  cudaSetDevice(c->device);
  if (c->batcher) loop_batcher_destroy(c->batcher);
  if (c->pool) {
    for (cudaStream_t s : c->pool->all) cudaStreamDestroy(s);
    delete c->pool;
  }
  for (Lane* l : c->lanes) lane_delete(l);
  DevBuf* bufs[] = {&c->d_keys, &c->d_vals, &c->d_ref, &c->d_ref_len, &c->d_counters, &c->d_msg, &c->d_msg_off, &c->d_digest};
  for (DevBuf* b : bufs) b->release();
  for (DevBuf& b : c->d_build) b.release();
  if (c->ev0) cudaEventDestroy(c->ev0);
  if (c->ev1) cudaEventDestroy(c->ev1);
  if (c->st) cudaStreamDestroy(c->st);
  delete c;
}

const char* ppd_last_error(const ppd_ctx* c) { return c ? c->err.c_str() : "null context"; }
void ppd_last_stats(const ppd_ctx* c, ppd_stats* out) {
  if (c && out) *out = c->stats;
}
void ppd_free(void* p) {
  if (p && !out_pool().give_back(p)) free(p);
}
void* ppd_alloc_pinned(size_t n) {
  void* p = out_pool().take(n ? n : 1);
  return p ? p : malloc(n ? n : 1);
}

int ppd_keccak256_batch(ppd_ctx* c, const uint8_t* data, const uint64_t* offsets, size_t n, uint8_t* out32n) {
  return guarded(c, [&] {
    stats_reset(c);
    if (!n) return;
    size_t bytes = offsets[n];
    c->d_msg.reserve(bytes + 16);
    c->d_msg_off.reserve((n + 1) * 8);
    c->d_digest.reserve(n * 32);
    CUDA_OK(cudaMemcpyAsync(c->d_msg.p, data, bytes, cudaMemcpyHostToDevice, c->st));
    CUDA_OK(cudaMemcpyAsync(c->d_msg_off.p, offsets, (n + 1) * 8, cudaMemcpyHostToDevice, c->st));
    CUDA_OK(cudaEventRecord(c->ev0, c->st));
    launch_keccak256_batch(c->d_msg.as<uint8_t>(), c->d_msg_off.as<uint64_t>(), (uint32_t)n, c->d_digest.as<uint8_t>(), c->st);
    CUDA_OK(cudaGetLastError());
    CUDA_OK(cudaEventRecord(c->ev1, c->st));
    CUDA_OK(cudaMemcpyAsync(out32n, c->d_digest.p, n * 32, cudaMemcpyDeviceToHost, c->st));
    CUDA_OK(cudaStreamSynchronize(c->st));
    float ms = 0;
    CUDA_OK(cudaEventElapsedTime(&ms, c->ev0, c->ev1));
    c->stats.gpu_ms = ms;
    c->stats.key_hashes = n;
    for (size_t i = 0; i < n; i++) c->stats.key_permutations += (offsets[i + 1] - offsets[i]) / 136 + 1;
    c->stats.h2d_bytes = (double)(bytes + (n + 1) * 8);
    c->stats.d2h_bytes = (double)(n * 32);
    c->stats.kernel_launches = 1;
  });
}

static void replay_lane(Lane* L, unsigned what) {
  cudaStream_t st = L->st;
  if ((what & PPD_REPLAY_PARSE) && L->has_last_parse) {
    ParseEmit E = L->last_emit;
    E.nodes = L->d_nodes.as<NodeRec>(), E.key_pool = L->d_keys.as<uint8_t>(), E.val_pool = L->d_vals.as<uint8_t>();
    E.hash_pool = L->d_hashes.as<uint8_t>(), E.child_pool = L->d_children.as<uint32_t>(), E.accounts = L->d_accounts.as<AccountRec>();
    E.level = L->d_level.as<uint16_t>();
    CUDA_OK(cudaMemsetAsync(L->last_bounds.result, 0, 4 * PARSE_R_WORDS, st));
    launch_parse_bounds(L->last_bounds, st);
    launch_parse_scatter(L->last_bounds, L->last_ins_pos, st);
    launch_parse_tree(E.T, st);
    if (L->last_n_code) {
      launch_parse_code_list(E, st);
      launch_keccak256_ranges(E.T.wit, E.code_se, L->last_n_code, const_cast<uint8_t*>(E.code_digest), st);
    }
    if (L->last_val_bytes) CUDA_OK(cudaMemsetAsync(E.val_pool, 0, L->last_val_bytes, st));
    launch_parse_emit(E, st);
  }
  if ((what & PPD_REPLAY_HASH) && L->has_last) {
    CUDA_OK(cudaMemsetAsync(L->d_counters.p, 0, 32, st));
    if (L->last_msg_data)
      launch_keccak256_ranges(L->last_msg_data, L->last_msg_se, L->last_n_msgs, L->last_digest_out, st);
    else
      launch_keccak256_ranges(L->d_msg.as<uint8_t>(), L->d_msg_off.as<uint64_t>(), L->last_n_msgs, L->d_digest.as<uint8_t>(), st);
    for (size_t l = 0; l + 1 < L->last_level_start.size(); l++)
      launch_hash_level(L->last_view, L->d_order.as<uint32_t>(), L->last_level_start[l], L->last_level_start[l + 1], st);
  }
  if ((what & PPD_REPLAY_TXN) && L->has_last_txn) {
    const txn::View& v = L->last_txn;
    CUDA_OK(cudaMemsetAsync(v.touched, 0xff, 4ull * L->last_n_touched, st));
    CUDA_OK(cudaMemsetAsync(L->last_join.slot_owner, 0xff, 4ull * (L->last_join.table_mask + 1), st));
    CUDA_OK(cudaMemsetAsync(L->last_join.slot_best, 0, 4ull * (L->last_join.table_mask + 1), st));
    CUDA_OK(cudaMemsetAsync(v.pre_slot, 0xff, 4ull * (L->last_join.n_acct + 1), st));
    launch_txn_init(v, L->last_init, L->last_table_slots, st);
    launch_join(L->last_join, st);
    launch_txn_prep(v, L->last_ai, L->last_n_ops1, L->last_n_ops2, L->last_max_writes, st);
    launch_txn_loop(L->h_task, v, L->last_init.state_root, L->last_max_keys, st);
    CUDA_OK(cudaMemsetAsync(L->last_bins_tail, 0, 4ull * ORDER_MAX_BINS, st));
    launch_order_by_level_class(v.nodes, v.level, L->last_cap_tail, ORDER_MAX_BINS, L->last_okeys, L->last_bins_tail, L->d_order2.as<uint32_t>(), st,
                                L->last_init.n_nodes, &v.cur->n_nodes);
  }
  if ((what & PPD_REPLAY_HASH) && L->has_last) {
    for (size_t l = 0; l + 1 < L->last_level_start2.size(); l++)
      launch_hash_level(L->last_view, L->d_order2.as<uint32_t>(), L->last_level_start2[l], L->last_level_start2[l + 1], st);
  }
  if ((what & PPD_REPLAY_DUMP) && L->has_last_txn) {
    launch_ir_size(L->last_view, L->last_plan, L->last_n_ir, st);
    launch_ir_emit(L->last_view, L->last_plan, L->last_n_ir, L->d_out.as<uint8_t>(), st);
  }
  CUDA_OK(cudaGetLastError());
}

static const size_t REPLAY_LANES_MAX = 30;
size_t ppd_replay_lanes(const ppd_ctx* c) { return c ? std::min(std::min(c->last_lanes_used, c->lanes.size()), REPLAY_LANES_MAX) : 0; }
int ppd_replay_last(ppd_ctx* c, unsigned what, double* gpu_ms_out) {
  return guarded(c, [&] {
    size_t used = 0;
    const size_t n_lanes = ppd_replay_lanes(c);
    for (size_t w = 0; w < n_lanes; w++) {
      const Lane* L = c->lanes[w];
      used += ((what & PPD_REPLAY_PARSE) && L->has_last_parse) || ((what & PPD_REPLAY_HASH) && L->has_last) ||
              ((what & (PPD_REPLAY_TXN | PPD_REPLAY_DUMP)) && L->has_last_txn);
    }
    if (!used) fail(PPD_ERR_BAD_ARGUMENT, "nothing of the requested kind is resident");
    CUDA_OK(cudaEventRecord(c->ev0, c->st));
    for (size_t w = 0; w < n_lanes; w++) {
      Lane* L = c->lanes[w];
      CUDA_OK(cudaStreamWaitEvent(L->st, c->ev0, 0));
      replay_lane(L, what);
      CUDA_OK(cudaEventRecord(L->ev1, L->st));
    }
    for (size_t w = 0; w < n_lanes; w++) CUDA_OK(cudaStreamWaitEvent(c->st, c->lanes[w]->ev1, 0));
    CUDA_OK(cudaEventRecord(c->ev1, c->st));
    CUDA_OK(cudaStreamSynchronize(c->st));
    float ms = 0;
    CUDA_OK(cudaEventElapsedTime(&ms, c->ev0, c->ev1));
    if (gpu_ms_out) *gpu_ms_out = ms;
  });
}
int ppd_replay_last_hashing(ppd_ctx* c, double* gpu_ms_out) { return ppd_replay_last(c, PPD_REPLAY_HASH, gpu_ms_out); }
int ppd_replay_last_parse(ppd_ctx* c, double* gpu_ms_out) { return ppd_replay_last(c, PPD_REPLAY_PARSE, gpu_ms_out); }

int ppd_microbench(ppd_ctx* c, int variant, uint32_t blocks_per_sm, uint32_t iters, double* gpu_ms_out, double* units_out, uint32_t* digest_out) {
  return guarded(c, [&] {
    c->d_counters.reserve(64);
    CUDA_OK(cudaMemsetAsync(c->d_counters.p, 0, 64, c->st));
    uint32_t bt = 0;
    double per = 0;
    if (!launch_microbench(variant, c->d_counters.as<uint32_t>(), blocks_per_sm, iters, &bt, &per, c->st)) fail(PPD_ERR_BAD_ARGUMENT, "unknown microbench variant");
    CUDA_OK(cudaEventRecord(c->ev0, c->st));
    launch_microbench(variant, c->d_counters.as<uint32_t>(), blocks_per_sm, iters, &bt, &per, c->st);
    CUDA_OK(cudaGetLastError());
    CUDA_OK(cudaEventRecord(c->ev1, c->st));
    uint32_t out[4];
    CUDA_OK(cudaMemcpyAsync(out, c->d_counters.p, 16, cudaMemcpyDeviceToHost, c->st));
    CUDA_OK(cudaStreamSynchronize(c->st));
    float ms = 0;
    CUDA_OK(cudaEventElapsedTime(&ms, c->ev0, c->ev1));
    if (gpu_ms_out) *gpu_ms_out = ms;
    if (units_out) *units_out = per * (double)iters * (double)bt * 148.0 * (double)blocks_per_sm;
    if (digest_out) digest_out[0] = out[2], digest_out[1] = out[3];
  });
}

int ppd_compact_decode(ppd_ctx* c, const uint8_t* witness, size_t len, uint8_t** out, size_t* out_len) {
  return guarded(c, [&] {
    stats_reset(c);
    Lane* L = lane_of(c, 0);
    L->stats = ppd_stats{};
    Job& J = job_of(L, 1);
    BlockJob& b = J.blocks[0];
    if (len >= 0xffffffffull) fail(PPD_ERR_BAD_ARGUMENT, "witness larger than 4 GiB");
    b.compact = Span{witness, (uint32_t)len};
    if (!(gpu_parse_enabled() && gpu_pre_image(L, J, b, false))) {
      parse_witness(witness, len, b.wit);
      collect_witness_messages(J, b);
      J.kh.run(L);
      build_pre_image(J, b);
    }
    uint32_t sr = root_node_for(J, b, b.state_root);
    std::map<H256, uint32_t> storage_roots;
    b.storage.for_each([&](const H256Map::Entry& s) { storage_roots[s.first] = root_node_for(J, b, s.second); });
    sweep(L, J);
    c->stats = L->stats;
    Out o;
    o.u32(PPD_PRE_IMAGE_MAGIC);
    o.u8(b.wit.version);
    o.raw(J.ref.data() + 32ull * sr, 32);
    o.u32((uint32_t)storage_roots.size());
    for (auto& s : storage_roots) {
      o.raw(s.first.b, 32);
      o.raw(J.ref.data() + 32ull * s.second, 32);
    }
    o.u32((uint32_t)b.pre_code.size());
    for (auto& cd : b.pre_code) {
      o.raw(cd.first.b, 32);
      o.u32(cd.second.n);
    }
    o.u64(c->stats.nodes_hashed);
    o.u64(c->stats.node_permutations);
    *out = o.give(out_len);
  });
}

int ppd_blocks_decode_batch(ppd_ctx* c, const uint8_t* const* flats, const size_t* lens, size_t n, uint8_t** outs, size_t* out_lens,
                            int* statuses) {
  int rc = guarded(c, [&] { decode_blocks(c, flats, lens, n, outs, out_lens, statuses); });
  if (rc != PPD_OK && outs)
    for (size_t i = 0; i < n; i++) {
      if (outs[i]) ppd_free(outs[i]);
      outs[i] = nullptr;
      if (out_lens) out_lens[i] = 0;
    }
  return rc;
}

int ppd_blocks_decode_stream(ppd_ctx* c, const uint8_t* const* flats, const size_t* lens, size_t n, ppd_block_done_fn done, void* user) {
  if (!done) return PPD_ERR_BAD_ARGUMENT;
  std::vector<uint8_t*> outs(n, nullptr);
  std::vector<size_t> out_lens(n, 0);
  std::vector<int> statuses(n, PPD_OK);
  int rc = guarded(c, [&] { decode_blocks(c, flats, lens, n, outs.data(), out_lens.data(), statuses.data(), done, user); });
  for (size_t i = 0; i < n; i++)
    if (outs[i]) ppd_free(outs[i]);
  return rc;
}

int ppd_block_decode(ppd_ctx* c, const uint8_t* flat, size_t len, uint8_t** out, size_t* out_len) {
  int status = PPD_OK;
  int rc = guarded(c, [&] { decode_blocks(c, &flat, &len, 1, out, out_len, &status); });
  if (rc != PPD_OK && out && *out) {
    ppd_free(*out);
    *out = nullptr;
  }
  return rc != PPD_OK ? rc : status;
}

}

namespace {

void trie_root_sorted_dev(ppd_ctx* c, const uint8_t* d_keys, const uint64_t* d_val_off, const uint8_t* d_vals, size_t n_, uint8_t root_out[32], int base_depth = 0) {
  if (n_ == 0) {
    memcpy(root_out, EMPTY_TRIE_HASH, 32);
    return;
  }
  if (n_ >= 0x7fffffffull) fail(PPD_ERR_BAD_ARGUMENT, "at most 2^31 - 2 leaves per call");
  const uint32_t n = (uint32_t)n_;
  cudaStream_t st = c->st;
  const uint32_t n1 = (n + 1 + 63) / 64, n2 = (n1 + 63) / 64, n3 = (n2 + 63) / 64;
  enum { B_L, B_M, B_LINKA, B_LINKB, B_BIDX, B_TMP, B_SMALL, B_DEPTH, B_REP, B_CHILD, B_ORDER, B_NCHILD };
  DevBuf* D = c->d_build;
  D[B_L].reserve((size_t)n + 1 + 64);
  D[B_M].reserve((size_t)n1 + n2 + n3 + 192);
  D[B_LINKA].reserve(4ull * (n + 1));
  D[B_LINKB].reserve(4ull * (n + 1));
  D[B_BIDX].reserve(4ull * (n + 1));
  D[B_TMP].reserve(4ull * scan_tmp_words((size_t)n + 1));
  D[B_SMALL].reserve(16384);
  int8_t* L = D[B_L].as<int8_t>();
  int8_t* m1 = D[B_M].as<int8_t>();
  int8_t* m2 = m1 + ((n1 + 63) & ~63u);
  int8_t* m3 = m2 + ((n2 + 63) & ~63u);
  uint32_t* small = D[B_SMALL].as<uint32_t>();
  CUDA_OK(cudaMemsetAsync(small, 0, 16384, st));
  CUDA_OK(cudaEventRecord(c->ev0, st));
  launch_lcp(d_keys, n, L, small + 0, st, base_depth);
  launch_min64(L, n + 1, m1, n1, st);
  launch_min64(m1, n1, m2, n2, st);
  launch_min64(m2, n2, m3, n3, st);
  uint32_t* leader = D[B_LINKA].as<uint32_t>();
  uint32_t* flag = D[B_LINKB].as<uint32_t>();
  launch_leaders(L, m1, m2, m3, n, leader, flag, flag, st);
  uint32_t* bidx = D[B_BIDX].as<uint32_t>();
  exclusive_scan_u32(flag, bidx, n + 1, D[B_TMP].as<uint32_t>(), st);
  CUDA_OK(cudaGetLastError());
  uint32_t h_flags = 0, nb = 0;
  CUDA_OK(cudaMemcpyAsync(&h_flags, small, 4, cudaMemcpyDeviceToHost, st));
  CUDA_OK(cudaMemcpyAsync(&nb, bidx + n, 4, cudaMemcpyDeviceToHost, st));
  CUDA_OK(cudaStreamSynchronize(st));
  if (h_flags & BUILD_F_UNSORTED) fail(PPD_ERR_UNSORTED_KEYS, "keys are not strictly ascending");
  if (h_flags & BUILD_F_PREFIX) fail(PPD_ERR_BAD_ARGUMENT, "the keys of a sub-trie do not share their first base_depth nibbles");
  c->stats.kernel_launches += 11 + 3;

  D[B_DEPTH].reserve(2ull * nb + 64);
  D[B_REP].reserve(4ull * nb + 64);
  D[B_CHILD].reserve(64ull * nb + 64);
  D[B_ORDER].reserve(4ull * nb + 64);
  c->d_ref.reserve(32ull * ((size_t)n + nb));
  c->d_ref_len.reserve((size_t)n + nb);
  BuildView V;
  V.keys = d_keys;
  V.val_off = d_val_off;
  V.vals = d_vals;
  V.n = n;
  V.base_depth = base_depth;
  V.P = Pyramid{L, m1, m2, m3};
  V.leader = leader;
  V.bidx = bidx;
  V.depth = D[B_DEPTH].as<uint8_t>();
  V.ext_start = V.depth + nb + 32;
  V.rep = D[B_REP].as<uint32_t>();
  V.child = D[B_CHILD].as<uint32_t>();
  V.root_id = small + 1;
  V.flags = small + 0;
  V.ref =c->d_ref.as<uint8_t>();
  V.ref_len = c->d_ref_len.as<uint8_t>();
  V.root_out = reinterpret_cast<uint8_t*>(small + 8);
  V.counters = reinterpret_cast<unsigned long long*>(small + 2);
  D[B_NCHILD].reserve(4ull * nb + 64);
  uint32_t* nchild = D[B_NCHILD].as<uint32_t>();
  if (nb) CUDA_OK(cudaMemsetAsync(V.child, 0xff, 64ull * nb, st));
  if (nb) CUDA_OK(cudaMemsetAsync(nchild, 0, 4ull * nb, st));
  launch_branch_info(V, st);
  launch_child_count(leader, bidx, n, nchild, st);
  launch_depth_hist(V.depth, nchild, nb, small + 1024, st);
  std::vector<uint32_t> hist(1024), cursor(1024), start(1024);
  CUDA_OK(cudaMemcpyAsync(hist.data(), small + 1024, 4096, cudaMemcpyDeviceToHost, st));
  CUDA_OK(cudaStreamSynchronize(st));
  uint32_t acc = 0;
  for (int d = 63; d >= 0; d--)
    for (int k = 0; k < 16; k++) {
      cursor[16 * d + k] = start[16 * d + k] = acc;
      acc += hist[16 * d + k];
    }
  if (acc != nb) fail(PPD_ERR_CUDA, "branch histogram does not add up");
  CUDA_OK(cudaMemcpyAsync(small + 2048, cursor.data(), 4096, cudaMemcpyHostToDevice, st));
  uint32_t* order = D[B_ORDER].as<uint32_t>();
  launch_branch_scatter(V.depth, nchild, nb, small + 2048, order, st);
  launch_hash_sorted_leaves(V, st);
  c->stats.kernel_launches += 5;
  uint32_t levels = 1;
  for (int d = 63; d >= 0; d--) {
    uint32_t cnt = 0;
    for (int k = 0; k < 16; k++) cnt += hist[16 * d + k];
    if (cnt) {
      launch_hash_branch_level(V, order, start[16 * d], start[16 * d] + cnt, st);
      c->stats.kernel_launches++;
      levels++;
    }
  }
  CUDA_OK(cudaGetLastError());
  CUDA_OK(cudaEventRecord(c->ev1, st));
  uint32_t out[16];
  CUDA_OK(cudaMemcpyAsync(out, small, 64, cudaMemcpyDeviceToHost, st));
  CUDA_OK(cudaStreamSynchronize(st));
  if (out[0] & BUILD_F_SHORT_TOP) fail(PPD_ERR_BAD_ARGUMENT, "the sub-trie's top node encodes to fewer than 32 bytes: its parent embeds it, not its hash");
  memcpy(root_out, out + 8, 32);
  float ms = 0;
  CUDA_OK(cudaEventElapsedTime(&ms, c->ev0, c->ev1));
  unsigned long long cnt[3];
  memcpy(cnt, out + 2, 24);
  c->stats.gpu_ms += ms;
  c->stats.nodes_hashed += cnt[0];
  c->stats.node_permutations += cnt[1];
  c->stats.node_bytes += cnt[2];
  c->stats.arena_nodes += (uint64_t)n + nb;
  c->stats.levels += levels;
  c->stats.d2h_bytes += 64 + 4096 + 8;
}

}

extern "C" {

int ppd_trie_root_sorted_leaves_dev(ppd_ctx* c, const uint8_t* d_keys32, const uint64_t* d_val_off, const uint8_t* d_vals, size_t n,
                                    size_t vals_bytes, uint8_t root_out[32]) {
  (void)vals_bytes;
  return guarded(c, [&] {
    stats_reset(c);
    trie_root_sorted_dev(c, d_keys32, d_val_off, d_vals, n, root_out);
  });
}

int ppd_trie_subroot_sorted_leaves_dev(ppd_ctx* c, const uint8_t* d_keys32, const uint64_t* d_val_off, const uint8_t* d_vals, size_t n,
                                       size_t vals_bytes, uint32_t base_depth, uint8_t ref_out[32]) {
  (void)vals_bytes;
  return guarded(c, [&] {
    stats_reset(c);
    if (base_depth >= 64 || n == 0) fail(PPD_ERR_BAD_ARGUMENT, "a sub-trie needs leaves and a base depth below 64");
    trie_root_sorted_dev(c, d_keys32, d_val_off, d_vals, n, ref_out, (int)base_depth);
  });
}

int ppd_trie_root_from_children(ppd_ctx* c, const uint8_t* child_hashes16x32, uint32_t mask, uint8_t root_out[32]) {
  return guarded(c, [&] {
    stats_reset(c);
    mask &= 0xffffu;
    if (__builtin_popcount(mask) < 2) fail(PPD_ERR_BAD_ARGUMENT, "a branch has at least two children");
    NodeRec nodes[2];
    uint32_t kids[16], k = 0;
    for (uint32_t i = 0; i < 16; i++)
      if (mask & (1u << i)) kids[k++] = HASH_ID_BASE + i;
    nodes[0] = NodeRec{node_w0(NK_BRANCH, 0, 0), 0, mask, 0};
    nodes[1] = NodeRec{node_w0(NK_ROOT, 0, 0), 0, 0, 0};
    c->d_keys.reserve(4096), c->d_vals.reserve(4096), c->d_ref.reserve(4096), c->d_ref_len.reserve(256), c->d_counters.reserve(32);
    c->d_msg.reserve(4096);
    uint8_t* base = c->d_msg.as<uint8_t>();
    CUDA_OK(cudaMemcpyAsync(base, child_hashes16x32, 512, cudaMemcpyHostToDevice, c->st));
    CUDA_OK(cudaMemcpyAsync(base + 512, nodes, sizeof nodes, cudaMemcpyHostToDevice, c->st));
    CUDA_OK(cudaMemcpyAsync(base + 1024, kids, 4 * k, cudaMemcpyHostToDevice, c->st));
    CUDA_OK(cudaMemsetAsync(c->d_counters.p, 0, 32, c->st));
    ArenaView V{};
    V.nodes = reinterpret_cast<const NodeRec*>(base + 512), V.hash_pool = base, V.child_pool = reinterpret_cast<const uint32_t*>(base + 1024);
    V.key_pool = c->d_keys.as<uint8_t>(), V.val_pool = c->d_vals.as<uint8_t>(), V.accounts = nullptr;
    V.ref = c->d_ref.as<uint8_t>(), V.ref_len = c->d_ref_len.as<uint8_t>(), V.counters = c->d_counters.as<unsigned long long>();
    launch_hash_level(V, nullptr, 0, 1, c->st);
    launch_hash_level(V, nullptr, 1, 2, c->st);
    CUDA_OK(cudaGetLastError());
    CUDA_OK(cudaMemcpyAsync(root_out, V.ref + 32, 32, cudaMemcpyDeviceToHost, c->st));
    CUDA_OK(cudaStreamSynchronize(c->st));
    c->stats.nodes_hashed = 2, c->stats.kernel_launches = 2;
  });
}

int ppd_trie_root_sorted_leaves(ppd_ctx* c, const uint8_t* keys32, const uint64_t* val_off, const uint8_t* vals, size_t n,
                                uint8_t root_out[32]) {
  return guarded(c, [&] {
    stats_reset(c);
    if (!n) {
      trie_root_sorted_dev(c, nullptr, nullptr, nullptr, 0, root_out);
      return;
    }
    size_t vb = val_off[n];
    c->d_keys.reserve(32 * n);
    c->d_msg_off.reserve(8 * (n + 1));
    c->d_vals.reserve(vb + 64);
    CUDA_OK(cudaMemcpyAsync(c->d_keys.p, keys32, 32 * n, cudaMemcpyHostToDevice, c->st));
    CUDA_OK(cudaMemcpyAsync(c->d_msg_off.p, val_off, 8 * (n + 1), cudaMemcpyHostToDevice, c->st));
    CUDA_OK(cudaMemcpyAsync(c->d_vals.p, vals, vb, cudaMemcpyHostToDevice, c->st));
    c->stats.h2d_bytes += (double)(32 * n + 8 * (n + 1) + vb);
    trie_root_sorted_dev(c, c->d_keys.as<uint8_t>(), c->d_msg_off.as<uint64_t>(), c->d_vals.as<uint8_t>(), n, root_out);
  });
}

}
```

proof_protocol_decoder_b200/csrc/ppd_kernels.cu:

```cuda
#include <cstdint>

#include "arena.h"
#include "encode.cuh"
#include "keccak.cuh"
#include "ppd_kernels.h"

namespace ppd {

using namespace enc;

static constexpr uint32_t FULL = 0xffffffffu;

static constexpr uint32_t HASH_ID_BASE = 0x80000000u;
__device__ __forceinline__ const uint8_t* ref_ptr(const ArenaView& A, uint32_t id) {
  return id >= HASH_ID_BASE ? A.hash_pool + 32ull * (id - HASH_ID_BASE) : A.ref + 32ull * id;
}
__device__ __forceinline__ uint32_t ref_len_of(const ArenaView& A, uint32_t id) { return id >= HASH_ID_BASE ? 32u : (uint32_t)A.ref_len[id]; }


template <int B>
__global__ void __launch_bounds__(B) keccak256_batch_kernel(const uint8_t* __restrict__ data, const uint64_t* __restrict__ offsets,
                                                            uint32_t stride, uint32_t n, uint8_t* __restrict__ out) {
  __shared__ uint32_t smem[PPD_STAGE_WORDS * B];
  const uint32_t i = blockIdx.x * B + threadIdx.x;
  bool busy = i < n;
  Stage<B> s;
  s.init(smem);
  uint64_t a[25];
#pragma unroll
  for (int k = 0; k < 25; k++) a[k] = 0;
  const uint8_t* p = data;
  uint64_t left = 0;
  if (busy) {
    const uint64_t m_begin = offsets[(uint64_t)i * stride], m_end = offsets[(uint64_t)i * stride + 1];
    p = data + m_begin;
    left = m_end - m_begin;
  }
  for (;;) {
    bool last = false;
    if (busy) {
      while (s.bytes() < 136 && left) {
        uint32_t take = left < 128 ? (uint32_t)left : 128u;
        emit_bytes(s, p, take);
        p += take;
        left -= take;
      }
      last = s.bytes() < 136;
      if (last) s.pad();
      absorb_stage<B>(a, s);
    }
    if (!__any_sync(FULL, busy)) break;
    keccak_f1600(a);
    if (busy) {
      if (last) {
        uint4 x, y;
        digest_words(a, x, y);
        uint4* o = reinterpret_cast<uint4*>(out + 32ull * i);
        o[0] = x, o[1] = y;
        busy = false;
      } else {
        s.consume_block();
      }
    }
  }
}


template <int B>
__global__ void __launch_bounds__(B, 4) hash_level_kernel(ArenaView A, const uint32_t* __restrict__ order, uint32_t begin, uint32_t end) {
  __shared__ uint32_t smem[PPD_STAGE_WORDS * B];
  const uint32_t slot = begin + blockIdx.x * B + threadIdx.x;
  uint32_t hashed = 0, perms = 0, enc_bytes = 0;
  bool busy = false, force_hash = false;
  uint32_t id = 0;
  uint4 rec = make_uint4(NK_HASH, 0, 0, 0);
  uint32_t payload = 0, nunit = 0, total = 0, unit = 0;
  uint32_t v0 = 0, v1 = 0;
#define KIND (rec.x & 0xff)
#define NIB_START ((rec.x >> 8) & 0xff)
#define NIB_LEN ((rec.x >> 16) & 0xff)
#define MY_REF (A.ref + 32ull * id)

  if (slot < end) {
    id = order ? __ldg(order + slot) : slot;
    rec = __ldg(reinterpret_cast<const uint4*>(A.nodes) + id);
    const uint8_t* copy_src = nullptr;
    busy = true;
    switch (KIND) {
      case NK_LEAF: {
        const uint8_t* val = A.val_pool + rec.z;
        v0 = rec.w;
        v1 = (v0 == 1 && __ldg(val) < 0x80) ? 0 : len_prefix_size(v0);
        payload = hex_prefix_str_size(NIB_LEN) + v1 + v0;
        nunit = 1 + ((v0 + 127) >> 7);
        break;
      }
      case NK_LEAF_ACCOUNT: {
        const AccountRec* acc = A.accounts + rec.z;
        uint32_t nn = u256_sig_bytes(acc->nonce);
        uint32_t nb = u256_sig_bytes(acc->balance);
        uint32_t apayload = u256_str_size(acc->nonce, nn) + u256_str_size(acc->balance, nb) + 66;
        v0 = len_prefix_size(apayload) + apayload;
        v1 = nn | (nb << 8) | (apayload << 16);
        payload = hex_prefix_str_size(NIB_LEN) + len_prefix_size(v0) + v0;
        nunit = 2;
        break;
      }
      case NK_EXT: {
        uint32_t clen = ref_len_of(A, rec.z);
        payload = hex_prefix_str_size(NIB_LEN) + (clen == 32 ? 33 : clen);
        nunit = 1;
        break;
      }
      case NK_BRANCH: {
        const uint32_t* ch = A.child_pool + rec.y;
        const uint32_t mask = rec.z & 0xffff;
        const uint32_t k = __popc(mask);
        uint32_t cid[16];
#pragma unroll
        for (int j = 0; j < 16; j++) cid[j] = (uint32_t)j < k ? __ldg(ch + j) : NODE_EMPTY;
        payload = 17 - k;
        uint32_t hashed_kids = 0;
#pragma unroll
        for (int j = 0; j < 16; j++) {
          uint32_t cl = cid[j] == NODE_EMPTY ? 0u : ref_len_of(A, cid[j]);
          payload += cl == 32 ? 33u : cl;
          hashed_kids |= (cl == 32 ? 1u : 0u) << j;
        }
        v0 = mask;
        v1 = hashed_kids << 16;
        nunit = 1 + (k + 2) / 3;
        break;
      }
      case NK_ROOT: {
        force_hash = true;
        if (rec.z != NODE_EMPTY && ref_len_of(A, rec.z) == 32) copy_src = ref_ptr(A, rec.z);
        nunit = 1;
        break;
      }
      default:
        busy = false;
        break;
    }
    if (copy_src) {
      const uint4* src = reinterpret_cast<const uint4*>(copy_src);
      uint4 x = __ldcg(src), y = __ldcg(src + 1);
      uint4* o = reinterpret_cast<uint4*>(MY_REF);
      o[0] = x;
      o[1] = y;
      A.ref_len[id] = 32;
      busy = false;
    }
    total = KIND == NK_ROOT ? 0 : len_prefix_size(payload) + payload;
  }
  const bool inline_ref = !force_hash && total < 32;

  Stage<B> s;
  s.init(smem);
  uint64_t a[25];
#pragma unroll
  for (int k = 0; k < 25; k++) a[k] = 0;

  for (;;) {
    bool permute = false, last = false;
    if (busy) {
      while (s.bytes() < 136 && unit < nunit) {
        switch (KIND) {
          case NK_LEAF:
            if (unit == 0) {
              emit_len_prefix(s, payload, 0xc0, 0xf7);
              emit_hex_prefix_str(s, A.key_pool + rec.y, NIB_START, NIB_LEN, 1);
              if (v1) emit_len_prefix(s, v0, 0x80, 0xb7);
            } else {
              uint32_t off = (unit - 1) << 7;
              emit_bytes(s, A.val_pool + rec.z + off, min(128u, v0 - off));
            }
            break;
          case NK_LEAF_ACCOUNT: {
            const AccountRec* acc = A.accounts + rec.z;
            if (unit == 0) {
              emit_len_prefix(s, payload, 0xc0, 0xf7);
              emit_hex_prefix_str(s, A.key_pool + rec.y, NIB_START, NIB_LEN, 1);
              emit_len_prefix(s, v0, 0x80, 0xb7);
              emit_len_prefix(s, v1 >> 16, 0xc0, 0xf7);
              emit_u256_str(s, acc->nonce, v1 & 0xff);
            } else {
              emit_u256_str(s, acc->balance, (v1 >> 8) & 0xff);
              uint32_t src = acc->storage_src;
              emit_ref_at(s, src == NODE_EMPTY ? acc->storage_root : A.ref + 32ull * src, 32);
              emit_ref_at(s, acc->code_hash, 32);
            }
            break;
          }
          case NK_EXT:
            emit_len_prefix(s, payload, 0xc0, 0xf7);
            emit_hex_prefix_str(s, A.key_pool + rec.y, NIB_START, NIB_LEN, 0);
            emit_ref_at(s, ref_ptr(A, rec.z), ref_len_of(A, rec.z));
            break;
          case NK_BRANCH:
            if (unit == 0) {
              emit_len_prefix(s, payload, 0xc0, 0xf7);
            } else {
              const uint32_t* ch = A.child_pool + rec.y;
              uint32_t j0 = (v1 >> 8) & 0xff, next_slot = v1 & 0xff;
              uint32_t nib[3], cid[3];
              uint4 x[3], y[3];
#pragma unroll
              for (int t = 0; t < 3; t++) {
                nib[t] = v0 ? (uint32_t)__ffs(v0) - 1 : 16u;
                v0 &= v0 - 1;
                cid[t] = nib[t] < 16 ? __ldg(ch + j0 + t) : 0u;
              }
#pragma unroll
              for (int t = 0; t < 3; t++) {
                if (nib[t] < 16) {
                  const uint4* q = reinterpret_cast<const uint4*>(ref_ptr(A, cid[t]));
                  x[t] = __ldcg(q), y[t] = __ldcg(q + 1);
                }
              }
#pragma unroll
              for (int t = 0; t < 3; t++) {
                if (nib[t] < 16) {
                  emit_empty_run(s, nib[t] - next_slot);
                  emit_ref(s, x[t], y[t], ((v1 >> (16 + j0 + t)) & 1) ? 32u : ref_len_of(A, cid[t]));
                  next_slot = nib[t] + 1;
                }
              }
              if (v0 == 0) emit_empty_run(s, 17 - next_slot);
              v1 = (v1 & 0xffff0000u) | ((j0 + 3) << 8) | next_slot;
            }
            break;
          default:
            if (rec.z == NODE_EMPTY)
              s.put_byte(0x80);
            else
              emit_ref_at(s, ref_ptr(A, rec.z), ref_len_of(A, rec.z));
            break;
        }
        unit++;
      }
      if (inline_ref) {
        uint4 x, y;
        inline_ref_words(s, total, x, y);
        uint4* o = reinterpret_cast<uint4*>(MY_REF);
        o[0] = x, o[1] = y;
        A.ref_len[id] = (uint8_t)total;
        busy = false;
      } else {
        last = s.bytes() < 136;
        if (last) s.pad();
        absorb_stage<B>(a, s);
        permute = true;
      }
    }
    if (!__any_sync(FULL, permute)) break;
    keccak_f1600(a);
    if (permute) {
      perms++;
      if (last) {
        uint4 x, y;
        digest_words(a, x, y);
        uint4* o = reinterpret_cast<uint4*>(MY_REF);
        o[0] = x, o[1] = y;
        A.ref_len[id] = 32;
        hashed = 1;
        enc_bytes = KIND == NK_ROOT ? (rec.z == NODE_EMPTY ? 1u : ref_len_of(A, rec.z)) : total;
        busy = false;
      } else {
        s.consume_block();
      }
    }
  }
  add_counters(A.counters, hashed, perms, enc_bytes);
#undef KIND
#undef NIB_START
#undef NIB_LEN
#undef MY_REF
}


static constexpr int KB = 128;

void launch_keccak256_batch(const uint8_t* data, const uint64_t* offsets, uint32_t n, uint8_t* out, cudaStream_t st) {
  if (!n) return;
  keccak256_batch_kernel<KB><<<(n + KB - 1) / KB, KB, 0, st>>>(data, offsets, 1, n, out);
}
void launch_keccak256_ranges(const uint8_t* data, const uint64_t* begin_end, uint32_t n, uint8_t* out, cudaStream_t st) {
  if (!n) return;
  keccak256_batch_kernel<KB><<<(n + KB - 1) / KB, KB, 0, st>>>(data, begin_end, 2, n, out);
}
static constexpr int OS_THREADS = 256, OS_PER = 8;

__device__ __forceinline__ uint32_t node_class(const NodeRec& r) {
  const uint32_t kind = r.w0 & 0xff;
  if (kind == NK_BRANCH) return 40 + ((__popc(r.a1 & 0xffff) - 1) & 15);
  if (kind == NK_ROOT) return 56;
  uint32_t perms = 1;
  if (kind == NK_LEAF) {
    const uint32_t nl = (r.w0 >> 16) & 0xff;
    perms = ((nl < 2 ? 1 : 2 + (nl >> 1)) + r.a2 + 6) / 136 + 1;
  }
  return kind * 8 + (perms > 8 ? 7 : perms - 1);
}

__global__ void __launch_bounds__(OS_THREADS) order_hist_kernel(const NodeRec* __restrict__ nodes, const uint16_t* __restrict__ level, uint32_t n,
                                                                uint32_t n_bins, uint16_t* __restrict__ keys, uint32_t* __restrict__ bins,
                                                                uint32_t first, const uint32_t* __restrict__ n_dev) {
  extern __shared__ uint32_t sh[];
  if (n_dev) n = min(n, *n_dev - first);
  if (blockIdx.x * (OS_THREADS * OS_PER) >= n) return;
  for (uint32_t k = threadIdx.x; k < n_bins; k += OS_THREADS) sh[k] = 0;
  __syncthreads();
  const uint32_t base = blockIdx.x * (OS_THREADS * OS_PER);
#pragma unroll
  for (int q = 0; q < OS_PER; q++) {
    const uint32_t i = base + q * OS_THREADS + threadIdx.x;
    if (i < n) {
      const uint32_t key = min((uint32_t)level[first + i] * 64u + node_class(nodes[first + i]), n_bins - 1);
      keys[i] = (uint16_t)key;
      atomicAdd(&sh[key], 1u);
    }
  }
  __syncthreads();
  for (uint32_t k = threadIdx.x; k < n_bins; k += OS_THREADS)
    if (sh[k]) atomicAdd(&bins[k], sh[k]);
}

__global__ void __launch_bounds__(1024) order_scan_kernel(uint32_t* __restrict__ bins, uint32_t n_bins) {
  __shared__ uint32_t warp_sums[32];
  __shared__ uint32_t carry;
  if (threadIdx.x == 0) carry = 0;
  __syncthreads();
  for (uint32_t base = 0; base < n_bins; base += 1024) {
    const uint32_t i = base + threadIdx.x;
    const uint32_t v = i < n_bins ? bins[i] : 0u;
    uint32_t incl = v;
    for (int off = 1; off < 32; off <<= 1) {
      uint32_t t = __shfl_up_sync(0xffffffffu, incl, off);
      if ((threadIdx.x & 31) >= (uint32_t)off) incl += t;
    }
    if ((threadIdx.x & 31) == 31) warp_sums[threadIdx.x >> 5] = incl;
    __syncthreads();
    if (threadIdx.x < 32) {
      uint32_t ws = warp_sums[threadIdx.x], wi = ws;
      for (int off = 1; off < 32; off <<= 1) {
        uint32_t t = __shfl_up_sync(0xffffffffu, wi, off);
        if (threadIdx.x >= (uint32_t)off) wi += t;
      }
      warp_sums[threadIdx.x] = wi - ws;
    }
    __syncthreads();
    const uint32_t excl = carry + warp_sums[threadIdx.x >> 5] + incl - v;
    if (i < n_bins) bins[i] = excl;
    __syncthreads();
    if (threadIdx.x == 1023) carry = excl + v;
    __syncthreads();
  }
}

__global__ void __launch_bounds__(OS_THREADS) order_scatter_kernel(const uint16_t* __restrict__ keys, uint32_t n, uint32_t n_bins,
                                                                   uint32_t* __restrict__ cursor, uint32_t* __restrict__ order, uint32_t first,
                                                                   const uint32_t* __restrict__ n_dev) {
  extern __shared__ uint32_t sh[];
  if (n_dev) n = min(n, *n_dev - first);
  if (blockIdx.x * (OS_THREADS * OS_PER) >= n) return;
  for (uint32_t k = threadIdx.x; k < n_bins; k += OS_THREADS) sh[k] = 0;
  __syncthreads();
  const uint32_t base = blockIdx.x * (OS_THREADS * OS_PER);
  uint32_t key[OS_PER], rank[OS_PER];
#pragma unroll
  for (int q = 0; q < OS_PER; q++) {
    const uint32_t i = base + q * OS_THREADS + threadIdx.x;
    key[q] = i < n ? keys[i] : 0xffffffffu;
    rank[q] = i < n ? atomicAdd(&sh[key[q]], 1u) : 0u;
  }
  __syncthreads();
  for (uint32_t k = threadIdx.x; k < n_bins; k += OS_THREADS)
    if (sh[k]) sh[k] = atomicAdd(&cursor[k], sh[k]);
  __syncthreads();
#pragma unroll
  for (int q = 0; q < OS_PER; q++) {
    const uint32_t i = base + q * OS_THREADS + threadIdx.x;
    if (i < n) order[sh[key[q]] + rank[q]] = first + i;
  }
}

__global__ void copy_segments_kernel(CopyBatch B) {
  const uint32_t s = blockIdx.y;
  uint8_t* d = reinterpret_cast<uint8_t*>(B.dst[s]);
  const uint8_t* p = reinterpret_cast<const uint8_t*>(B.src[s]);
  const unsigned long long n = B.bytes[s];
  const unsigned long long tid = (unsigned long long)blockIdx.x * blockDim.x + threadIdx.x, nt = (unsigned long long)gridDim.x * blockDim.x;
  const uintptr_t both = reinterpret_cast<uintptr_t>(d) | reinterpret_cast<uintptr_t>(p);
  unsigned long long done = 0;
  if ((both & 15) == 0) {
    const unsigned long long nv = n / 16;
    for (unsigned long long i = tid; i < nv; i += nt) reinterpret_cast<uint4*>(d)[i] = reinterpret_cast<const uint4*>(p)[i];
    done = nv * 16;
  } else if ((both & 3) == 0) {
    const unsigned long long nv = n / 4;
    for (unsigned long long i = tid; i < nv; i += nt) reinterpret_cast<uint32_t*>(d)[i] = reinterpret_cast<const uint32_t*>(p)[i];
    done = nv * 4;
  }
  for (unsigned long long i = done + tid; i < n; i += nt) d[i] = p[i];
}
void launch_copy_segments(const CopyBatch& B, cudaStream_t st) {
  if (!B.n) return;
  unsigned long long most = 0;
  for (uint32_t k = 0; k < B.n; k++) most = B.bytes[k] > most ? B.bytes[k] : most;
  uint32_t gx = (uint32_t)((most + 16 * 256 * 4 - 1) / (16 * 256 * 4));
  gx = gx < 1 ? 1 : (gx > 32 ? 32 : gx);
  copy_segments_kernel<<<dim3(gx, B.n), 256, 0, st>>>(B);
}
__global__ void store_u32x2_kernel(uint32_t* dst, uint32_t a, uint32_t b) { dst[0] = a, dst[1] = b; }
void launch_store_u32x2(uint32_t* dst, uint32_t a, uint32_t b, cudaStream_t st) { store_u32x2_kernel<<<1, 1, 0, st>>>(dst, a, b); }

void launch_order_by_level_class(const NodeRec* nodes, const uint16_t* level, uint32_t n, uint32_t n_bins, uint16_t* keys, uint32_t* bins,
                                 uint32_t* order, cudaStream_t st, uint32_t first, const uint32_t* n_dev) {
  if (!n) return;
  const uint32_t blocks = (n + OS_THREADS * OS_PER - 1) / (OS_THREADS * OS_PER);
  order_hist_kernel<<<blocks, OS_THREADS, 4 * n_bins, st>>>(nodes, level, n, n_bins, keys, bins, first, n_dev);
  order_scan_kernel<<<1, 1024, 0, st>>>(bins, n_bins);
  order_scatter_kernel<<<blocks, OS_THREADS, 4 * n_bins, st>>>(keys, n, n_bins, bins, order, first, n_dev);
}

void launch_hash_level(const ArenaView& A, const uint32_t* order, uint32_t begin, uint32_t end, cudaStream_t st) {
  if (end <= begin) return;
  uint32_t n = end - begin;
  hash_level_kernel<KB><<<(n + KB - 1) / KB, KB, 0, st>>>(A, order, begin, end);
}

}
```

proof_protocol_decoder_b200/csrc/ppd_kernels.h:

```cpp
#pragma once
#include <cuda_runtime.h>

#include <cstdint>

#include "arena.h"
#include "txn_core.h"

namespace ppd {

void launch_keccak256_batch(const uint8_t* data, const uint64_t* offsets, uint32_t n, uint8_t* out, cudaStream_t st);
void launch_keccak256_ranges(const uint8_t* data, const uint64_t* begin_end, uint32_t n, uint8_t* out, cudaStream_t st);
void launch_hash_level(const ArenaView& A, const uint32_t* order, uint32_t begin, uint32_t end, cudaStream_t st);
static const uint32_t ORDER_MAX_BINS = 4096;
void launch_order_by_level_class(const NodeRec* nodes, const uint16_t* level, uint32_t n, uint32_t n_bins, uint16_t* keys, uint32_t* bins,
                                 uint32_t* order, cudaStream_t st, uint32_t first = 0, const uint32_t* n_dev = nullptr);

struct CopyBatch {
  static const uint32_t MAX = 16;
  void* dst[MAX];
  const void* src[MAX];
  unsigned long long bytes[MAX];
  uint32_t n = 0;
};
void launch_copy_segments(const CopyBatch& B, cudaStream_t st);
void launch_store_u32x2(uint32_t* dst, uint32_t a, uint32_t b, cudaStream_t st);

struct Pyramid {
  const int8_t *L, *m1, *m2, *m3;
};

enum : uint32_t {
  BUILD_F_UNSORTED = 1,
  BUILD_F_PREFIX = 2,
  BUILD_F_SHORT_TOP = 4,
};

struct BuildView {
  const uint8_t* keys;
  const uint64_t* val_off;
  const uint8_t* vals;
  uint32_t n;
  int base_depth;
  Pyramid P;
  const uint32_t* leader;
  const uint32_t* bidx;
  uint8_t* depth;
  uint8_t* ext_start;
  uint32_t* rep;
  uint32_t* child;
  uint32_t* root_id;
  uint32_t* flags;
  uint8_t* ref;
  uint8_t* ref_len;
  uint8_t* root_out;
  unsigned long long* counters;
};

size_t scan_tmp_words(size_t n);
void exclusive_scan_u32(const uint32_t* in, uint32_t* out, uint32_t n, uint32_t* tmp, cudaStream_t st);
void launch_lcp(const uint8_t* keys, uint32_t n, int8_t* L, uint32_t* flags, cudaStream_t st, int base_depth = 0);
void launch_min64(const int8_t* in, uint32_t n_in, int8_t* out, uint32_t n_out, cudaStream_t st);
void launch_leaders(const int8_t* L, const int8_t* m1, const int8_t* m2, const int8_t* m3, uint32_t n, uint32_t* link_a, uint32_t* link_b,
                    uint32_t* flag, cudaStream_t st);
void launch_branch_info(const BuildView& V, cudaStream_t st);
void launch_child_count(const uint32_t* leader, const uint32_t* bidx, uint32_t n, uint32_t* nchild, cudaStream_t st);
void launch_depth_hist(const uint8_t* depth, const uint32_t* nchild, uint32_t nb, uint32_t* hist, cudaStream_t st);
void launch_branch_scatter(const uint8_t* depth, const uint32_t* nchild, uint32_t nb, uint32_t* cursor, uint32_t* order, cudaStream_t st);
void launch_hash_sorted_leaves(const BuildView& V, cudaStream_t st);
void launch_hash_branch_level(const BuildView& V, const uint32_t* order, uint32_t begin, uint32_t end, cudaStream_t st);

struct IrDumpPlanView {
  const uint32_t* touched;
  const uint32_t* touched_begin;
  const uint32_t* seg_a;
  const uint32_t* seg_b;
  const uint32_t* seg_begin;
  const uint32_t* seg_end;
  const uint32_t* seg_c;
  const uint8_t* flat;
  const uint8_t* lit;
  const uint64_t* ir_base;
  const uint64_t* big_off;
  const uint32_t* big_cap;
  uint32_t* big_scratch;
  uint32_t* seg_off;
  uint32_t* ir_size;
  uint32_t* ir_flag;
  uint32_t* ir_nuniq;
  uint32_t* u_node;
  uint32_t* u_size;
  uint32_t* u_off;
};
void launch_ir_size(const ArenaView& A, const IrDumpPlanView& P, uint32_t n_ir, cudaStream_t st);
static const uint32_t MARK_SLOTS = 16;
static const uint32_t IR_SET_MAX_UNIQ = 4096;
void launch_ir_emit(const ArenaView& A, const IrDumpPlanView& P, uint32_t n_ir, uint8_t* out, cudaStream_t st);

static const uint32_t PARSE_TILE = 4096;
static const uint32_t PARSE_ERR = 0xffffff00u;
enum {
  PARSE_R_END = 0,
  PARSE_R_NINS = 1,
  PARSE_R_FLAG = 2,
  PARSE_R_HEIGHT = 3,
  PARSE_R_ROOT = 4,
  PARSE_R_ROOT_ID = 5,
  PARSE_R_NKEYED = 6,
  PARSE_R_TOTALS = 8,
  PARSE_R_WORDS = 16
};
enum { PARSE_WHY_DECODE = 1, PARSE_WHY_STACK = 2, PARSE_WHY_NOT_CANONICAL = 3, PARSE_WHY_LEAF_KIND = 4, PARSE_WHY_KEY = 5 };
enum {
  PARSE_C_NODE = 0,
  PARSE_C_HASH = 1,
  PARSE_C_KEY = 2,
  PARSE_C_VAL = 3,
  PARSE_C_CHILD = 4,
  PARSE_C_ACCT = 5,
  PARSE_C_CODE = 6,
  PARSE_N_CNT = 7
};
struct ParseBounds {
  const uint8_t* wit;
  uint32_t n;
  uint32_t n_tiles, group_tiles, n_groups;
  uint32_t* exit1;
  uint16_t* step1;
  uint32_t* exit2;
  uint32_t* group_entry;
  uint32_t* tile_entry;
  uint32_t* bitmap;
  uint32_t* tile_count;
  uint32_t* tile_base;
  uint32_t* scan_tmp;
  uint32_t* result;
};
struct ParseTree {
  const uint8_t* wit;
  uint32_t n, n_ins;
  const uint32_t* ins_pos;
  uint32_t* meta;
  uint8_t* knib;
  uint32_t* delta;
  uint32_t* hb;
  int16_t *h16, *m0, *m1, *m2, *m3;
  uint32_t* parent;
  uint32_t* info;
  uint32_t* aux0;
  uint32_t* keyed;
  uint32_t *pending, *lvlmax;
  uint32_t *cnt, *scn;
  size_t cnt_stride;
  uint32_t* scan_tmp;
  uint32_t* result;
};
struct ParseEmit {
  ParseTree T;
  NodeRec* nodes;
  uint16_t* level;
  uint8_t *key_pool, *val_pool, *hash_pool;
  uint32_t* child_pool;
  AccountRec* accounts;
  uint32_t* acct_list;
  uint64_t* code_se;
  uint32_t* code_list;
  const uint8_t* code_digest;
  uint32_t n_keyed;
};
size_t parse_scan_tmp_words(size_t n, uint32_t K);
uint32_t launch_parse_bounds(const ParseBounds& B, cudaStream_t st);
void launch_parse_scatter(const ParseBounds& B, uint32_t* ins_pos, cudaStream_t st);
uint32_t launch_parse_tree(const ParseTree& T, cudaStream_t st);
void launch_parse_code_list(const ParseEmit& E, cudaStream_t st);
void launch_parse_emit(const ParseEmit& E, cudaStream_t st);

void launch_txn_msgs(const txn::View& v, uint64_t* se, cudaStream_t st);
void launch_txn_init(const txn::View& v, const txn::Cursors& init, uint32_t table_slots, cudaStream_t st);
void launch_join(const txn::JoinView& j, cudaStream_t st);
uint32_t launch_txn_prep(const txn::View& v, const txn::AcctInit& a, uint32_t n_ops1, uint32_t n_ops2, uint32_t max_writes, cudaStream_t st);
static const uint32_t LOOP_BATCH_MAX = 12;
uint32_t launch_txn_loops(const txn::LoopTask* tasks, uint32_t n, uint32_t max_txns, bool any_shared, cudaStream_t st);
uint32_t txn_loop_uses_shared(uint32_t max_keys);
uint32_t launch_txn_loop(txn::LoopTask* slot, const txn::View& v, uint32_t initial_state, uint32_t max_keys, cudaStream_t st);
void launch_acct_export(const txn::View& v, const txn::JoinView& j, txn::AcctExport* out, cudaStream_t st);

bool launch_microbench(int variant, uint32_t* out, uint32_t blocks_per_sm, uint32_t iters, uint32_t* block_threads, double* units_per_thread_iter,
                       cudaStream_t st);

}
```

Measured before the change: 1.460 billion.

## Replace per-level hash launches with one dependency-driven sweep kernel

New measurement: 476.5 million (median of 6 runs). -67.4%, worse.

```diff
diff --git a/proof_protocol_decoder_b200/csrc/gpu_txn.cu b/proof_protocol_decoder_b200/csrc/gpu_txn.cu
--- a/proof_protocol_decoder_b200/csrc/gpu_txn.cu
+++ b/proof_protocol_decoder_b200/csrc/gpu_txn.cu
@@ -282,13 +282,11 @@
   L->stats.kernel_launches += 3, L->stats.d2h_bytes += 4.0 * ORDER_MAX_BINS;
 }
 
-void levels_from_bins(const uint32_t* bins, uint32_t n, std::vector<uint32_t>& level_start) {
-  level_start.assign(1, 0);
-  for (uint32_t l = 0; l < ORDER_MAX_BINS / 64; l++) {
-    const uint32_t end = bins[64 * l + 63];
-    level_start.push_back(end);
-    if (end >= n) break;
-  }
+uint32_t levels_from_bins(const uint32_t* bins, uint32_t n) {
+  if (bins[ORDER_MAX_BINS - 1] != bins[ORDER_MAX_BINS - 2]) return 0;
+  uint32_t l = 0;
+  while (bins[64 * l + 63] < n) l++;
+  return l + 1;
 }
 
 }
@@ -426,22 +424,25 @@
   lane_copy_flush(L);
   CUDA_OK(cudaMemsetAsync(d_touched, 0xff, 4ull * n_touched, st));
   v.txns = d_txns, v.touched = d_touched, v.seg_a = d_seg_a, v.seg_b = d_seg_b;
-  std::vector<uint32_t> level_pre, level_tail;
-  levels_from_bins(H.h_bins, n_pre, level_pre);
+  const uint32_t levels_pre = levels_from_bins(H.h_bins, n_pre);
+  if (!levels_pre) {
+    if (getenv("PPD_TIMING")) fprintf(stderr, "[ppd] pre-image deeper than %u levels: host path\n", ORDER_MAX_BINS / 64);
+    L->stats = stats0;
+    L->has_last_parse = false;
+    return GPU_BLOCK_DECLINED;
+  }
   L->d_ref.reserve(32ull * v.cap_nodes);
   L->d_ref_len.reserve(v.cap_nodes);
-  L->d_counters.reserve(32);
-  CUDA_OK(cudaMemsetAsync(L->d_counters.p, 0, 32, st));
+  L->d_counters.reserve(64);
+  CUDA_OK(cudaMemsetAsync(L->d_counters.p, 0, SWEEP_COUNTER_BYTES, st));
   ArenaView V;
   V.nodes = v.nodes, V.key_pool = v.key_pool, V.val_pool = v.val_pool, V.hash_pool = v.hash_pool, V.child_pool = v.child_pool;
   V.accounts = v.accounts, V.ref = L->d_ref.as<uint8_t>(), V.ref_len = L->d_ref_len.as<uint8_t>();
   V.counters = L->d_counters.as<unsigned long long>();
   trace_mark(L, "plan_up");
   CUDA_OK(cudaEventRecord(L->ev0, st));
-  for (size_t l = 0; l + 1 < level_pre.size(); l++) {
-    launch_hash_level(V, L->d_order.as<uint32_t>(), level_pre[l], level_pre[l + 1], st);
-    L->stats.kernel_launches++, L->stats.level_launches++;
-  }
+  launch_hash_sweep(V, L->d_order.as<uint32_t>(), 0, n_pre, sweep_ticket(V, 0), st);
+  L->stats.kernel_launches++, L->stats.level_launches++;
   CUDA_OK(cudaEventRecord(L->ev1, st));
   trace_mark(L, "pre_hashed");
   H.j.ref = V.ref;
@@ -553,13 +554,11 @@
     pt.lap("t:dummies");
   }
   const uint32_t n_total = h_cur->n_nodes, n_tail = n_total - n_pre;
-  levels_from_bins(H.h_bins + ORDER_MAX_BINS, n_tail, level_tail);
+  const uint32_t levels_tail = levels_from_bins(H.h_bins + ORDER_MAX_BINS, n_tail);
   trace_mark(L, "host_resumed");
   CUDA_OK(cudaEventRecord(L->ev0, st));
-  for (size_t l = 0; l + 1 < level_tail.size(); l++) {
-    launch_hash_level(V, L->d_order2.as<uint32_t>(), level_tail[l], level_tail[l + 1], st);
-    L->stats.kernel_launches++, L->stats.level_launches++;
-  }
+  launch_hash_sweep(V, L->d_order2.as<uint32_t>(), n_pre, n_tail, sweep_ticket(V, 1), st);
+  L->stats.kernel_launches++, L->stats.level_launches++;
   CUDA_OK(cudaEventRecord(L->ev1, st));
   trace_mark(L, "tail_hashed");
   CUDA_OK(cudaEventRecord(L->ev_loop0, st));
@@ -570,8 +569,8 @@
   uint32_t* h_sizes = J.plan.data();
   unsigned long long* h_counters = reinterpret_cast<unsigned long long*>(H.h_bins);
   lane_copy(L, h_sizes, d_ir_size, 8ull * n_ir);
-  lane_copy(L, h_counters, L->d_counters.p, 24);
-  L->stats.kernel_launches += 1, L->stats.d2h_bytes += 8.0 * n_ir + 24;
+  lane_copy(L, h_counters, L->d_counters.p, 32);
+  L->stats.kernel_launches += 1, L->stats.d2h_bytes += 8.0 * n_ir + 32;
   trace_mark(L, "ir_sized");
   lane_sync(L);
   pt.lap("t:sweep+size");
@@ -582,9 +581,10 @@
     CUDA_OK(cudaEventElapsedTime(&ms, L->ev_loop0, L->ev_loop1));
     L->stats.dump_gpu_ms += ms;
   }
+  if (h_counters[3]) fail(PPD_ERR_CUDA, "the node sweep gave up waiting for a node's children (the (level, class) order is broken)");
   L->stats.nodes_hashed += h_counters[0], L->stats.node_permutations += h_counters[1], L->stats.node_bytes += h_counters[2];
   L->stats.arena_nodes += n_total;
-  L->stats.levels += level_pre.size() + level_tail.size() - 2;
+  L->stats.levels += levels_pre + levels_tail;
   for (size_t m = 0; m < T.traces.size(); m++) {
     const txn::TxnTrace& tr = T.traces[m];
     L->stats.key_permutations += 1 + tr.n_reads + tr.n_writes + ((tr.flags & txn::TRF_MIN_KEYS) ? tr.n_writes : 0);
@@ -593,7 +593,7 @@
   L->stats.marks_on_gpu += T.n_items;
   L->stats.txn_loops_on_gpu += 1;
   L->has_last = true, L->last_view = V;
-  L->last_level_start = level_pre, L->last_level_start2 = level_tail, L->last_n_msgs = T.n_msgs;
+  L->last_n_pre = n_pre, L->last_n_tail = n_tail, L->last_n_msgs = T.n_msgs;
   L->last_msg_data = d_flat, L->last_msg_se = H.se, L->last_digest_out = v.key_pool + H.B.dig_base;
   L->last_txn = H.v, L->last_join = H.j, L->last_ai = H.ai, L->last_init = init, L->last_table_slots = H.table_slots;
   L->last_n_ops1 = T.n_ops1, L->last_n_ops2 = T.n_ops2, L->last_max_writes = max_writes, L->last_n_touched = n_touched, L->last_max_keys = T.max_ops;
diff --git a/proof_protocol_decoder_b200/csrc/host_pipeline.h b/proof_protocol_decoder_b200/csrc/host_pipeline.h
--- a/proof_protocol_decoder_b200/csrc/host_pipeline.h
+++ b/proof_protocol_decoder_b200/csrc/host_pipeline.h
@@ -61,7 +61,7 @@
   Job* job = nullptr;
   bool has_last = false;
   ArenaView last_view{};
-  std::vector<uint32_t> last_level_start, last_level_start2;
+  uint32_t last_n_pre = 0, last_n_tail = 0;
   uint32_t last_n_msgs = 0;
   const uint8_t* last_msg_data = nullptr;
   const uint64_t* last_msg_se = nullptr;
diff --git a/proof_protocol_decoder_b200/csrc/ppd_host.cu b/proof_protocol_decoder_b200/csrc/ppd_host.cu
--- a/proof_protocol_decoder_b200/csrc/ppd_host.cu
+++ b/proof_protocol_decoder_b200/csrc/ppd_host.cu
@@ -197,9 +197,6 @@
 #endif
   uint32_t n_levels = 0;
   for (uint32_t i = 0; i < n; i++) n_levels = std::max<uint32_t>(n_levels, A.level[i] + 1u);
-  std::vector<uint32_t> level_start(n_levels + 1, 0);
-  for (uint32_t i = 0; i < n; i++) level_start[A.level[i] + 1u]++;
-  for (uint32_t l = 0; l < n_levels; l++) level_start[l + 1] += level_start[l];
   const bool device_order = 64u * n_levels <= ORDER_MAX_BINS;
   PVec<uint32_t>& order = J.order;
   if (!device_order) {
@@ -235,7 +232,7 @@
   c->d_accounts.reserve_keep(sizeof(AccountRec) * A.accounts.size() + 16, sizeof(AccountRec) * R.accounts, c->st);
   c->d_ref.reserve(32ull * n);
   c->d_ref_len.reserve(n);
-  c->d_counters.reserve(32);
+  c->d_counters.reserve(64);
   auto up = [&](DevBuf& d, const void* src, size_t bytes, size_t resident = 0) {
     if (bytes <= resident) return;
     CUDA_OK(cudaMemcpyAsync(d.as<uint8_t>() + resident, (const uint8_t*)src + resident, bytes - resident, cudaMemcpyHostToDevice, c->st));
@@ -259,7 +256,7 @@
   up(c->d_hashes, A.hash_pool.data(), A.hash_pool.size(), R.hashes);
   up(c->d_children, A.child_pool.data(), 4ull * A.child_pool.size(), 4ull * R.children);
   up(c->d_accounts, A.accounts.data(), sizeof(AccountRec) * A.accounts.size(), sizeof(AccountRec) * R.accounts);
-  CUDA_OK(cudaMemsetAsync(c->d_counters.p, 0, 32, c->st));
+  CUDA_OK(cudaMemsetAsync(c->d_counters.p, 0, SWEEP_COUNTER_BYTES, c->st));
   ArenaView V;
   V.nodes = c->d_nodes.as<NodeRec>();
   V.key_pool = c->d_keys.as<uint8_t>();
@@ -271,18 +268,16 @@
   V.ref_len = c->d_ref_len.as<uint8_t>();
   V.counters = c->d_counters.as<unsigned long long>();
   CUDA_OK(cudaEventRecord(c->ev0, c->st));
-  for (uint32_t l = 0; l < n_levels; l++) {
-    launch_hash_level(V, c->d_order.as<uint32_t>(), level_start[l], level_start[l + 1], c->st);
-    c->stats.kernel_launches++;
-    c->stats.level_launches++;
-  }
+  launch_hash_sweep(V, c->d_order.as<uint32_t>(), 0, n, sweep_ticket(V, 0), c->st);
+  c->stats.kernel_launches++;
+  c->stats.level_launches++;
   CUDA_OK(cudaGetLastError());
   CUDA_OK(cudaEventRecord(c->ev1, c->st));
-  unsigned long long counters[3] = {0, 0, 0};
+  unsigned long long counters[4] = {0, 0, 0, 0};
   c->has_last = true;
   c->last_view = V;
-  c->last_level_start = level_start;
-  c->last_level_start2.clear();
+  c->last_n_pre = n;
+  c->last_n_tail = 0;
   c->last_msg_data = nullptr;
   c->has_last_txn = false;
   c->last_n_msgs = (uint32_t)J.kh.lens.size();
@@ -291,8 +286,9 @@
     CUDA_OK(cudaMemcpyAsync(J.ref.data(), c->d_ref.p, 32ull * n, cudaMemcpyDeviceToHost, c->st));
     CUDA_OK(cudaMemcpyAsync(J.ref_len.data(), c->d_ref_len.p, n, cudaMemcpyDeviceToHost, c->st));
   }
-  CUDA_OK(cudaMemcpyAsync(counters, c->d_counters.p, 24, cudaMemcpyDeviceToHost, c->st));
+  CUDA_OK(cudaMemcpyAsync(counters, c->d_counters.p, 32, cudaMemcpyDeviceToHost, c->st));
   lane_sync(c);
+  if (counters[3]) fail(PPD_ERR_CUDA, "the node sweep gave up waiting for a node's children (the (level, class) order is broken)");
   float ms = 0;
   CUDA_OK(cudaEventElapsedTime(&ms, c->ev0, c->ev1));
   c->stats.gpu_ms += ms;
@@ -600,13 +596,12 @@
     launch_parse_emit(E, st);
   }
   if ((what & PPD_REPLAY_HASH) && L->has_last) {
-    CUDA_OK(cudaMemsetAsync(L->d_counters.p, 0, 32, st));
+    CUDA_OK(cudaMemsetAsync(L->d_counters.p, 0, SWEEP_COUNTER_BYTES, st));
     if (L->last_msg_data)
       launch_keccak256_ranges(L->last_msg_data, L->last_msg_se, L->last_n_msgs, L->last_digest_out, st);
     else
       launch_keccak256_ranges(L->d_msg.as<uint8_t>(), L->d_msg_off.as<uint64_t>(), L->last_n_msgs, L->d_digest.as<uint8_t>(), st);
-    for (size_t l = 0; l + 1 < L->last_level_start.size(); l++)
-      launch_hash_level(L->last_view, L->d_order.as<uint32_t>(), L->last_level_start[l], L->last_level_start[l + 1], st);
+    launch_hash_sweep(L->last_view, L->d_order.as<uint32_t>(), 0, L->last_n_pre, sweep_ticket(L->last_view, 0), st);
   }
   if ((what & PPD_REPLAY_TXN) && L->has_last_txn) {
     const txn::View& v = L->last_txn;
@@ -623,8 +618,7 @@
                                 L->last_init.n_nodes, &v.cur->n_nodes);
   }
   if ((what & PPD_REPLAY_HASH) && L->has_last) {
-    for (size_t l = 0; l + 1 < L->last_level_start2.size(); l++)
-      launch_hash_level(L->last_view, L->d_order2.as<uint32_t>(), L->last_level_start2[l], L->last_level_start2[l + 1], st);
+    launch_hash_sweep(L->last_view, L->d_order2.as<uint32_t>(), L->last_n_pre, L->last_n_tail, sweep_ticket(L->last_view, 1), st);
   }
   if ((what & PPD_REPLAY_DUMP) && L->has_last_txn) {
     launch_ir_size(L->last_view, L->last_plan, L->last_n_ir, st);
@@ -916,23 +910,25 @@
       if (mask & (1u << i)) kids[k++] = HASH_ID_BASE + i;
     nodes[0] = NodeRec{node_w0(NK_BRANCH, 0, 0), 0, mask, 0};
     nodes[1] = NodeRec{node_w0(NK_ROOT, 0, 0), 0, 0, 0};
-    c->d_keys.reserve(4096), c->d_vals.reserve(4096), c->d_ref.reserve(4096), c->d_ref_len.reserve(256), c->d_counters.reserve(32);
+    c->d_keys.reserve(4096), c->d_vals.reserve(4096), c->d_ref.reserve(4096), c->d_ref_len.reserve(256), c->d_counters.reserve(64);
     c->d_msg.reserve(4096);
     uint8_t* base = c->d_msg.as<uint8_t>();
     CUDA_OK(cudaMemcpyAsync(base, child_hashes16x32, 512, cudaMemcpyHostToDevice, c->st));
     CUDA_OK(cudaMemcpyAsync(base + 512, nodes, sizeof nodes, cudaMemcpyHostToDevice, c->st));
     CUDA_OK(cudaMemcpyAsync(base + 1024, kids, 4 * k, cudaMemcpyHostToDevice, c->st));
-    CUDA_OK(cudaMemsetAsync(c->d_counters.p, 0, 32, c->st));
+    CUDA_OK(cudaMemsetAsync(c->d_counters.p, 0, SWEEP_COUNTER_BYTES, c->st));
     ArenaView V{};
     V.nodes = reinterpret_cast<const NodeRec*>(base + 512), V.hash_pool = base, V.child_pool = reinterpret_cast<const uint32_t*>(base + 1024);
     V.key_pool = c->d_keys.as<uint8_t>(), V.val_pool = c->d_vals.as<uint8_t>(), V.accounts = nullptr;
     V.ref = c->d_ref.as<uint8_t>(), V.ref_len = c->d_ref_len.as<uint8_t>(), V.counters = c->d_counters.as<unsigned long long>();
-    launch_hash_level(V, nullptr, 0, 1, c->st);
-    launch_hash_level(V, nullptr, 1, 2, c->st);
+    launch_hash_sweep(V, nullptr, 0, 2, sweep_ticket(V, 0), c->st);
     CUDA_OK(cudaGetLastError());
+    unsigned long long counters[4];
     CUDA_OK(cudaMemcpyAsync(root_out, V.ref + 32, 32, cudaMemcpyDeviceToHost, c->st));
+    CUDA_OK(cudaMemcpyAsync(counters, c->d_counters.p, 32, cudaMemcpyDeviceToHost, c->st));
     CUDA_OK(cudaStreamSynchronize(c->st));
-    c->stats.nodes_hashed = 2, c->stats.kernel_launches = 2;
+    if (counters[3]) fail(PPD_ERR_CUDA, "the node sweep gave up waiting for a node's children");
+    c->stats.nodes_hashed = 2, c->stats.kernel_launches = 1;
   });
 }
 
diff --git a/proof_protocol_decoder_b200/csrc/ppd_kernels.cu b/proof_protocol_decoder_b200/csrc/ppd_kernels.cu
--- a/proof_protocol_decoder_b200/csrc/ppd_kernels.cu
+++ b/proof_protocol_decoder_b200/csrc/ppd_kernels.cu
@@ -15,7 +15,6 @@
 __device__ __forceinline__ const uint8_t* ref_ptr(const ArenaView& A, uint32_t id) {
   return id >= HASH_ID_BASE ? A.hash_pool + 32ull * (id - HASH_ID_BASE) : A.ref + 32ull * id;
 }
-__device__ __forceinline__ uint32_t ref_len_of(const ArenaView& A, uint32_t id) { return id >= HASH_ID_BASE ? 32u : (uint32_t)A.ref_len[id]; }
 
 
 template <int B>
@@ -66,95 +65,50 @@
 }
 
 
+static constexpr uint32_t SWEEP_WAIT_NS = 1000000000u;
+static constexpr uint32_t SWEEP_SLEEP_NS = 500;
+
+__device__ __forceinline__ uint32_t ld_relaxed_u8(const uint8_t* p) {
+  uint16_t v;
+  asm volatile("ld.relaxed.gpu.global.u8 %0, [%1];" : "=h"(v) : "l"(p) : "memory");
+  return v;
+}
+__device__ __forceinline__ uint32_t ld_relaxed_u32(const uint32_t* p) {
+  uint32_t v;
+  asm volatile("ld.relaxed.gpu.global.u32 %0, [%1];" : "=r"(v) : "l"(p) : "memory");
+  return v;
+}
+__device__ __forceinline__ void st_release_u8(uint8_t* p, uint32_t v) {
+  asm volatile("st.release.gpu.global.u8 [%0], %1;" ::"l"(p), "h"((uint16_t)v) : "memory");
+}
+__device__ __forceinline__ void fence_acq_rel_gpu() { asm volatile("fence.acq_rel.gpu;" ::: "memory"); }
+__device__ __forceinline__ uint32_t globaltimer_lo() {
+  uint32_t t;
+  asm volatile("mov.u32 %0, %%globaltimer_lo;" : "=r"(t));
+  return t;
+}
+__device__ __forceinline__ uint32_t ref_len_now(const ArenaView& A, uint32_t id) { return id >= HASH_ID_BASE ? 32u : ld_relaxed_u8(A.ref_len + id); }
+
 template <int B>
-__global__ void __launch_bounds__(B, 4) hash_level_kernel(ArenaView A, const uint32_t* __restrict__ order, uint32_t begin, uint32_t end) {
+__global__ void __launch_bounds__(B, 4) hash_sweep_kernel(ArenaView A, const uint32_t* __restrict__ order, uint32_t id_first, uint32_t n,
+                                                          uint32_t* __restrict__ ticket) {
+  enum : uint32_t { IDLE = 0, WAIT = 1, BUSY = 2 };
   __shared__ uint32_t smem[PPD_STAGE_WORDS * B];
-  const uint32_t slot = begin + blockIdx.x * B + threadIdx.x;
+  const uint32_t lane = threadIdx.x & 31;
+  uint32_t* wait_flag = reinterpret_cast<uint32_t*>(A.counters + 3);
   uint32_t hashed = 0, perms = 0, enc_bytes = 0;
-  bool busy = false, force_hash = false;
-  uint32_t id = 0;
+  uint32_t phase = IDLE;
+  bool drained = false;
+  uint32_t id = 0, t0 = 0;
   uint4 rec = make_uint4(NK_HASH, 0, 0, 0);
   uint32_t payload = 0, nunit = 0, total = 0, unit = 0;
   uint32_t v0 = 0, v1 = 0;
+  bool inline_ref = false;
 #define KIND (rec.x & 0xff)
 #define NIB_START ((rec.x >> 8) & 0xff)
 #define NIB_LEN ((rec.x >> 16) & 0xff)
 #define MY_REF (A.ref + 32ull * id)
 
-  if (slot < end) {
-    id = order ? __ldg(order + slot) : slot;
-    rec = __ldg(reinterpret_cast<const uint4*>(A.nodes) + id);
-    const uint8_t* copy_src = nullptr;
-    busy = true;
-    switch (KIND) {
-      case NK_LEAF: {
-        const uint8_t* val = A.val_pool + rec.z;
-        v0 = rec.w;
-        v1 = (v0 == 1 && __ldg(val) < 0x80) ? 0 : len_prefix_size(v0);
-        payload = hex_prefix_str_size(NIB_LEN) + v1 + v0;
-        nunit = 1 + ((v0 + 127) >> 7);
-        break;
-      }
-      case NK_LEAF_ACCOUNT: {
-        const AccountRec* acc = A.accounts + rec.z;
-        uint32_t nn = u256_sig_bytes(acc->nonce);
-        uint32_t nb = u256_sig_bytes(acc->balance);
-        uint32_t apayload = u256_str_size(acc->nonce, nn) + u256_str_size(acc->balance, nb) + 66;
-        v0 = len_prefix_size(apayload) + apayload;
-        v1 = nn | (nb << 8) | (apayload << 16);
-        payload = hex_prefix_str_size(NIB_LEN) + len_prefix_size(v0) + v0;
-        nunit = 2;
-        break;
-      }
-      case NK_EXT: {
-        uint32_t clen = ref_len_of(A, rec.z);
-        payload = hex_prefix_str_size(NIB_LEN) + (clen == 32 ? 33 : clen);
-        nunit = 1;
-        break;
-      }
-      case NK_BRANCH: {
-        const uint32_t* ch = A.child_pool + rec.y;
-        const uint32_t mask = rec.z & 0xffff;
-        const uint32_t k = __popc(mask);
-        uint32_t cid[16];
-#pragma unroll
-        for (int j = 0; j < 16; j++) cid[j] = (uint32_t)j < k ? __ldg(ch + j) : NODE_EMPTY;
-        payload = 17 - k;
-        uint32_t hashed_kids = 0;
-#pragma unroll
-        for (int j = 0; j < 16; j++) {
-          uint32_t cl = cid[j] == NODE_EMPTY ? 0u : ref_len_of(A, cid[j]);
-          payload += cl == 32 ? 33u : cl;
-          hashed_kids |= (cl == 32 ? 1u : 0u) << j;
-        }
-        v0 = mask;
-        v1 = hashed_kids << 16;
-        nunit = 1 + (k + 2) / 3;
-        break;
-      }
-      case NK_ROOT: {
-        force_hash = true;
-        if (rec.z != NODE_EMPTY && ref_len_of(A, rec.z) == 32) copy_src = ref_ptr(A, rec.z);
-        nunit = 1;
-        break;
-      }
-      default:
-        busy = false;
-        break;
-    }
-    if (copy_src) {
-      const uint4* src = reinterpret_cast<const uint4*>(copy_src);
-      uint4 x = __ldcg(src), y = __ldcg(src + 1);
-      uint4* o = reinterpret_cast<uint4*>(MY_REF);
-      o[0] = x;
-      o[1] = y;
-      A.ref_len[id] = 32;
-      busy = false;
-    }
-    total = KIND == NK_ROOT ? 0 : len_prefix_size(payload) + payload;
-  }
-  const bool inline_ref = !force_hash && total < 32;
-
   Stage<B> s;
   s.init(smem);
   uint64_t a[25];
@@ -162,8 +116,116 @@
   for (int k = 0; k < 25; k++) a[k] = 0;
 
   for (;;) {
+    const uint32_t idle = __ballot_sync(FULL, phase == IDLE);
+    if (idle == FULL) {
+      if (drained) break;
+      uint32_t base = 0;
+      if (lane == 0) base = atomicAdd(ticket, 32u);
+      base = __shfl_sync(FULL, base, 0);
+      if (base >= n) break;
+      drained = base + 32 >= n;
+      if (base + lane < n) {
+        id = order ? __ldg(order + base + lane) : id_first + base + lane;
+        rec = __ldg(reinterpret_cast<const uint4*>(A.nodes) + id);
+        phase = WAIT;
+        t0 = globaltimer_lo();
+      }
+    }
+    if (phase == WAIT) {
+      bool ready = true, deps = true;
+      const uint8_t* copy_src = nullptr;
+      switch (KIND) {
+        case NK_LEAF: {
+          const uint8_t* val = A.val_pool + rec.z;
+          v0 = rec.w;
+          v1 = (v0 == 1 && __ldg(val) < 0x80) ? 0 : len_prefix_size(v0);
+          payload = hex_prefix_str_size(NIB_LEN) + v1 + v0;
+          nunit = 1 + ((v0 + 127) >> 7);
+          deps = false;
+          break;
+        }
+        case NK_LEAF_ACCOUNT: {
+          const AccountRec* acc = A.accounts + rec.z;
+          const uint32_t src = acc->storage_src;
+          ready = src == NODE_EMPTY || ref_len_now(A, src) != 0;
+          if (ready) {
+            uint32_t nn = u256_sig_bytes(acc->nonce);
+            uint32_t nb = u256_sig_bytes(acc->balance);
+            uint32_t apayload = u256_str_size(acc->nonce, nn) + u256_str_size(acc->balance, nb) + 66;
+            v0 = len_prefix_size(apayload) + apayload;
+            v1 = nn | (nb << 8) | (apayload << 16);
+            payload = hex_prefix_str_size(NIB_LEN) + len_prefix_size(v0) + v0;
+            nunit = 2;
+          }
+          break;
+        }
+        case NK_EXT: {
+          const uint32_t clen = ref_len_now(A, rec.z);
+          ready = clen != 0;
+          payload = hex_prefix_str_size(NIB_LEN) + (clen == 32 ? 33 : clen);
+          nunit = 1;
+          break;
+        }
+        case NK_BRANCH: {
+          const uint32_t* ch = A.child_pool + rec.y;
+          const uint32_t mask = rec.z & 0xffff;
+          const uint32_t k = __popc(mask);
+          uint32_t cid[16];
+#pragma unroll
+          for (int j = 0; j < 16; j++) cid[j] = (uint32_t)j < k ? __ldg(ch + j) : NODE_EMPTY;
+          uint32_t pl = 17 - k;
+          uint32_t hashed_kids = 0;
+#pragma unroll
+          for (int j = 0; j < 16; j++) {
+            const uint32_t cl = cid[j] == NODE_EMPTY ? 0u : ref_len_now(A, cid[j]);
+            ready = ready && (cid[j] == NODE_EMPTY || cl != 0);
+            pl += cl == 32 ? 33u : cl;
+            hashed_kids |= (cl == 32 ? 1u : 0u) << j;
+          }
+          payload = pl;
+          v0 = mask;
+          v1 = hashed_kids << 16;
+          nunit = 1 + (k + 2) / 3;
+          break;
+        }
+        case NK_ROOT: {
+          v0 = rec.z == NODE_EMPTY ? 1u : ref_len_now(A, rec.z);
+          ready = v0 != 0;
+          if (rec.z != NODE_EMPTY && v0 == 32) copy_src = ref_ptr(A, rec.z);
+          nunit = 1;
+          break;
+        }
+        default:
+          ready = false;
+          phase = IDLE;
+          break;
+      }
+      if (ready) {
+        if (deps) fence_acq_rel_gpu();
+        if (copy_src) {
+          const uint4* src = reinterpret_cast<const uint4*>(copy_src);
+          uint4 x = __ldcg(src), y = __ldcg(src + 1);
+          uint4* o = reinterpret_cast<uint4*>(MY_REF);
+          o[0] = x;
+          o[1] = y;
+          st_release_u8(A.ref_len + id, 32);
+          phase = IDLE;
+        } else {
+          total = KIND == NK_ROOT ? 0 : len_prefix_size(payload) + payload;
+          inline_ref = KIND != NK_ROOT && total < 32;
+          unit = 0;
+          s.init(smem);
+#pragma unroll
+          for (int k = 0; k < 25; k++) a[k] = 0;
+          phase = BUSY;
+        }
+      } else if (phase == WAIT && (globaltimer_lo() - t0 > SWEEP_WAIT_NS || ld_relaxed_u32(wait_flag))) {
+        atomicOr(wait_flag, 1u);
+        phase = IDLE;
+      }
+    }
     bool permute = false, last = false;
-    if (busy) {
+    if (phase == BUSY) {
       while (s.bytes() < 136 && unit < nunit) {
         switch (KIND) {
           case NK_LEAF:
@@ -192,11 +254,13 @@
             }
             break;
           }
-          case NK_EXT:
+          case NK_EXT: {
+            const uint32_t clen = payload - hex_prefix_str_size(NIB_LEN);
             emit_len_prefix(s, payload, 0xc0, 0xf7);
             emit_hex_prefix_str(s, A.key_pool + rec.y, NIB_START, NIB_LEN, 0);
-            emit_ref_at(s, ref_ptr(A, rec.z), ref_len_of(A, rec.z));
+            emit_ref_at(s, ref_ptr(A, rec.z), clen == 33 ? 32u : clen);
             break;
+          }
           case NK_BRANCH:
             if (unit == 0) {
               emit_len_prefix(s, payload, 0xc0, 0xf7);
@@ -222,7 +286,7 @@
               for (int t = 0; t < 3; t++) {
                 if (nib[t] < 16) {
                   emit_empty_run(s, nib[t] - next_slot);
-                  emit_ref(s, x[t], y[t], ((v1 >> (16 + j0 + t)) & 1) ? 32u : ref_len_of(A, cid[t]));
+                  emit_ref(s, x[t], y[t], ((v1 >> (16 + j0 + t)) & 1) ? 32u : ref_len_now(A, cid[t]));
                   next_slot = nib[t] + 1;
                 }
               }
@@ -234,7 +298,7 @@
             if (rec.z == NODE_EMPTY)
               s.put_byte(0x80);
             else
-              emit_ref_at(s, ref_ptr(A, rec.z), ref_len_of(A, rec.z));
+              emit_ref_at(s, ref_ptr(A, rec.z), v0);
             break;
         }
         unit++;
@@ -244,8 +308,8 @@
         inline_ref_words(s, total, x, y);
         uint4* o = reinterpret_cast<uint4*>(MY_REF);
         o[0] = x, o[1] = y;
-        A.ref_len[id] = (uint8_t)total;
-        busy = false;
+        st_release_u8(A.ref_len + id, total);
+        phase = IDLE;
       } else {
         last = s.bytes() < 136;
         if (last) s.pad();
@@ -253,7 +317,10 @@
         permute = true;
       }
     }
-    if (!__any_sync(FULL, permute)) break;
+    if (!__any_sync(FULL, permute)) {
+      if (__any_sync(FULL, phase == WAIT)) __nanosleep(SWEEP_SLEEP_NS);
+      continue;
+    }
     keccak_f1600(a);
     if (permute) {
       perms++;
@@ -262,10 +329,10 @@
         digest_words(a, x, y);
         uint4* o = reinterpret_cast<uint4*>(MY_REF);
         o[0] = x, o[1] = y;
-        A.ref_len[id] = 32;
-        hashed = 1;
-        enc_bytes = KIND == NK_ROOT ? (rec.z == NODE_EMPTY ? 1u : ref_len_of(A, rec.z)) : total;
-        busy = false;
+        st_release_u8(A.ref_len + id, 32);
+        hashed++;
+        enc_bytes += KIND == NK_ROOT ? v0 : total;
+        phase = IDLE;
       } else {
         s.consume_block();
       }
@@ -424,10 +491,10 @@
   order_scatter_kernel<<<blocks, OS_THREADS, 4 * n_bins, st>>>(keys, n, n_bins, bins, order, first, n_dev);
 }
 
-void launch_hash_level(const ArenaView& A, const uint32_t* order, uint32_t begin, uint32_t end, cudaStream_t st) {
-  if (end <= begin) return;
-  uint32_t n = end - begin;
-  hash_level_kernel<KB><<<(n + KB - 1) / KB, KB, 0, st>>>(A, order, begin, end);
-}
-
-}
+void launch_hash_sweep(const ArenaView& A, const uint32_t* order, uint32_t id_first, uint32_t n, uint32_t* ticket, cudaStream_t st) {
+  if (!n) return;
+  if (cudaMemsetAsync(A.ref_len + id_first, 0, n, st) != cudaSuccess) return;
+  hash_sweep_kernel<KB><<<(n + KB - 1) / KB, KB, 0, st>>>(A, order, id_first, n, ticket);
+}
+
+}
diff --git a/proof_protocol_decoder_b200/csrc/ppd_kernels.h b/proof_protocol_decoder_b200/csrc/ppd_kernels.h
--- a/proof_protocol_decoder_b200/csrc/ppd_kernels.h
+++ b/proof_protocol_decoder_b200/csrc/ppd_kernels.h
@@ -10,7 +10,9 @@
 
 void launch_keccak256_batch(const uint8_t* data, const uint64_t* offsets, uint32_t n, uint8_t* out, cudaStream_t st);
 void launch_keccak256_ranges(const uint8_t* data, const uint64_t* begin_end, uint32_t n, uint8_t* out, cudaStream_t st);
-void launch_hash_level(const ArenaView& A, const uint32_t* order, uint32_t begin, uint32_t end, cudaStream_t st);
+static const size_t SWEEP_COUNTER_BYTES = 48;
+inline uint32_t* sweep_ticket(const ArenaView& A, int sweep) { return reinterpret_cast<uint32_t*>(A.counters + 4 + sweep); }
+void launch_hash_sweep(const ArenaView& A, const uint32_t* order, uint32_t id_first, uint32_t n, uint32_t* ticket, cudaStream_t st);
 static const uint32_t ORDER_MAX_BINS = 4096;
 void launch_order_by_level_class(const NodeRec* nodes, const uint16_t* level, uint32_t n, uint32_t n_bins, uint16_t* keys, uint32_t* bins,
                                  uint32_t* order, cudaStream_t st, uint32_t first = 0, const uint32_t* n_dev = nullptr);
```
